# team-charls/charls

Hardware: AMD Instinct MI355X
Metric: MPixels/s encode+decode, 4096x4096 8-bit gray, bit-exact vs CharLS (higher is better)
Workload: dtype u8

## Files before the change

charls_amd/csrc/device/scan_group_decode.hip:

```cpp
#pragma once
#include <hip/hip_runtime.h>

#include "scan_model.h"
#include "scan_fast_decode.hip"
#ifndef JLS_EMULATED
#include "scan_group_step.inc"
#endif

namespace jls {
namespace grp {

constexpr uint32_t kRingWords = 256;
constexpr uint32_t kRingBits = kRingWords * 32;
constexpr int kStepsPerCheck = 64;
constexpr uint32_t kMarginBits = kStepsPerCheck * 32 + 320;
constexpr int kMaxTableT3 = 1023;
constexpr uint32_t kPrepRing = 128;
constexpr uint32_t kPrepSlots = kPrepRing + 64;
constexpr uint32_t kPrepChunk = 64;
constexpr int kStepsPerLoop = 63;

template <typename S>
struct Layout
{
    static constexpr uint32_t kLutBytes = sizeof(S) == 1 ? 512 : 2 * kMaxTableT3 + 2;
    static constexpr uint32_t kRecords = 0;
    static constexpr uint32_t kRun = 2928;
    static constexpr uint32_t kRing = kRun + 48;
    static constexpr uint32_t kPrep = kRing + kRingWords * 4 + 8;
    static constexpr uint32_t kLine = kPrep + kPrepSlots * 8 + 24 + 16 - sizeof(S);
    static_assert(kPrep % 8 == 0 && (kLine + sizeof(S)) % 16 == 0, "alignment of the prepared entries and of sample 1 of the line");
};

__host__ __device__ constexpr uint32_t bank_spread(uint32_t bytes)
{
    return ((bytes + 127u) & ~127u) + 16u;
}

template <typename S>
__host__ __device__ constexpr uint32_t line_stride_bytes(uint32_t width)
{
    return ((width + 6) * (uint32_t)sizeof(S) + 15u) & ~15u;
}

template <typename S>
__host__ __device__ constexpr uint32_t region_bytes(uint32_t width, uint32_t lines = 1)
{
    return bank_spread(Layout<S>::kLine + lines * line_stride_bytes<S>(width));
}

template <typename S>
__host__ __device__ constexpr uint32_t workgroup_lds_bytes(uint32_t width, uint32_t scans_per_wave, uint32_t lines = 1)
{
    return Layout<S>::kLutBytes + scans_per_wave * region_bytes<S>(width, lines);
}

struct Record
{
    uint32_t a;
    uint32_t ncb;
};

struct PrepEntry
{
    uint32_t x, y;
};
JLS_DEV PrepEntry load_pair(uint32_t address)
{
    const uint64_t w = lds_load<uint64_t>(address);
    return PrepEntry{(uint32_t)w, (uint32_t)(w >> 32)};
}
JLS_DEV void store_pair(uint32_t address, const PrepEntry& e)
{
    lds_store<uint64_t>(address, ((uint64_t)e.y << 32) | e.x);
}

#ifndef JLS_EMULATED
JLS_DEV uint32_t abs_difference_plus(uint32_t a, uint32_t b, uint32_t c)
{
    uint32_t r;
    asm("v_sad_u32 %0, %1, %2, %3" : "=v"(r) : "v"(a), "v"(b), "v"(c));
    return r;
}
#else
JLS_DEV uint32_t abs_difference_plus(uint32_t a, uint32_t b, uint32_t c)
{
    return (a > b ? a - b : b - a) + c;
}
#endif

JLS_DEV uint32_t peek32(const uint32_t* ring, uint32_t p)
{
    const uint32_t wi = (p >> 5) & (kRingWords - 1);
    const uint64_t both = ((uint64_t)ring[wi + 1] << 32) | ring[wi];
    return (uint32_t)(both >> (p & 31));
}

JLS_DEV uint64_t ring_words_at(uint32_t ring_address, uint32_t p)
{
    const uint32_t at = ring_address + (bit_field(p, 5, 8) << 2);
    return ((uint64_t)lds_load<uint32_t>(at + 4) << 32) | lds_load<uint32_t>(at);
}

JLS_DEV uint32_t field(uint32_t w, int n)
{
    return (uint32_t)(((uint64_t)bit_reverse(w) << n) >> 32);
}

JLS_DEV uint32_t take_bits(const uint32_t* ring, uint32_t& p, int n)
{
    const uint32_t w = peek32(ring, p);
    p += (uint32_t)n;
    return field(w, n);
}

struct Producer
{
    const uint8_t* gbase;
    uint64_t u_next;
    uint64_t u_end;
    uint64_t u_begin;
    uint64_t u_marker;
    uint32_t produced;
    uint32_t prev_byte;
    bool ended;
};

JLS_DEV void put_bits(uint32_t* ring, uint32_t p, uint32_t v, int n)
{
    const uint32_t q = (p >> 5) & (kRingWords - 1);
    const int off = (int)(p & 31);
    const uint32_t rv = bit_reverse(v) >> (32 - n);
    atomicOr(&ring[q], rv << off);
    if (q < 2)
        atomicOr(&ring[kRingWords + q], rv << off);
    if (off + n > 32)
    {
        const uint32_t q2 = (q + 1) & (kRingWords - 1);
        atomicOr(&ring[q2], rv >> (32 - off));
        if (q2 < 2)
            atomicOr(&ring[kRingWords + q2], rv >> (32 - off));
    }
}

template <int G>
JLS_DEV void refill_bytewise(Producer& s, uint32_t* ring, bool want, int lane, int sub, uint64_t u0, const uint4& raw,
                             uint32_t next_first, uint32_t before)
{
    constexpr uint32_t kChunk = G * 16;
    const uint32_t words[4] = {raw.x, raw.y, raw.z, raw.w};
    const uint32_t last = words[3] >> 24;
    int nbits[16];
    uint32_t bytes[16];
    int marker_at = 16;
    uint32_t prev = before;
    int total = 0;
#pragma unroll
    for (int j = 0; j < 16; ++j)
    {
        const uint32_t b = (words[j >> 2] >> ((j & 3) * 8)) & 0xFFu;
        const uint64_t u = u0 + (uint64_t)j;
        bytes[j] = b;
        int n = 0;
        if (u == s.u_begin)
            prev = 0;
        if (want && u >= s.u_begin && u < s.u_end && marker_at == 16)
        {
            const uint32_t nb = j < 15 ? ((words[(j + 1) >> 2] >> (((j + 1) & 3) * 8)) & 0xFFu) : next_first;
            const bool is_marker = b == 0xFFu && (u + 1 >= s.u_end || (nb & 0x80u) != 0);
            if (is_marker)
                marker_at = j;
            else
                n = prev == 0xFFu ? 7 : 8;
        }
        nbits[j] = n;
        total += n;
        prev = b;
    }
    const unsigned long long markers = __ballot(marker_at < 16);
    const int group_base = lane - sub;
    const uint32_t group_markers = (uint32_t)(markers >> group_base) & (G == 32 ? 0xFFFFFFFFu : ((1u << (G & 31)) - 1u));
    const unsigned long long group_markers64 = G == 64 ? markers : (unsigned long long)group_markers;
    const int first_marker = group_markers64 ? __ffsll(group_markers64) - 1 : 64;
    if (sub > first_marker)
        total = 0;
    int inc = total;
    for (int delta = 1; delta < G; delta <<= 1)
    {
        const int up = __shfl_up(inc, delta);
        if (sub >= delta)
            inc += up;
    }
    uint32_t p = s.produced + (uint32_t)(inc - total);
    if (want && sub <= first_marker)
    {
#pragma unroll
        for (int j = 0; j < 16; ++j)
            if (nbits[j] != 0)
            {
                put_bits(ring, p, nbits[j] == 7 ? (bytes[j] & 0x7Fu) : bytes[j], nbits[j]);
                p += (uint32_t)nbits[j];
            }
    }
    const int chunk_bits = __shfl(inc, group_base + G - 1);
    const uint32_t chunk_last = __shfl(last, group_base + G - 1);
    const int marker_j = __shfl(marker_at, group_base + (first_marker < G ? first_marker : 0));
    JLS_LOCKSTEP();
    if (want)
    {
        s.produced += (uint32_t)chunk_bits;
        s.prev_byte = chunk_last;
        if (first_marker < G)
        {
            s.u_marker = s.u_next + (uint64_t)first_marker * 16 + (uint64_t)marker_j;
            s.ended = true;
        }
        s.u_next += kChunk;
        if (s.u_next >= s.u_end)
            s.ended = true;
    }
}

JLS_DEV uint32_t ff_bytes(uint32_t w)
{
    const uint32_t v = ~w;
    return ~((((v & 0x7F7F7F7Fu) + 0x7F7F7F7Fu) | v) | 0x7F7F7F7Fu);
}

template <int G>
JLS_DEV void refill(Producer& s, uint32_t* ring, bool want, int lane, int sub)
{
    constexpr uint32_t kChunk = G * 16;
    if (want)
    {
        const uint32_t first = (s.produced + 31) >> 5;
        for (uint32_t j = sub; j < kChunk / 4 + 2; j += G)
        {
            const uint32_t q = (first + j) & (kRingWords - 1);
            ring[q] = 0;
            if (q < 2)
                ring[kRingWords + q] = 0;
        }
    }
    JLS_LOCKSTEP();
    const uint64_t u0 = s.u_next + (uint64_t)sub * 16;
    uint4 raw = make_uint4(0, 0, 0, 0);
    uint32_t next_first = 0;
    if (want && u0 < s.u_end)
    {
        raw = *reinterpret_cast<const uint4*>(s.gbase + u0);
        if (u0 + 16 < s.u_end)
            next_first = s.gbase[u0 + 16];
    }
    const uint32_t last = raw.w >> 24;
    uint32_t before = __shfl_up(last, 1);
    if (sub == 0)
        before = s.prev_byte;
    const uint32_t z0 = ff_bytes(raw.x), z1 = ff_bytes(raw.y), z2 = ff_bytes(raw.z), z3 = ff_bytes(raw.w);
    const uint32_t marker_like = (((z0 << 8) & raw.x) | (((z1 << 8) | (z0 >> 24)) & raw.y) | (((z2 << 8) | (z1 >> 24)) & raw.z) |
                                  (((z3 << 8) | (z2 >> 24)) & raw.w) | ((z3 >> 24) & next_first)) & 0x80808080u;
    const bool inside = u0 >= s.u_begin && u0 + 17 <= s.u_end;
    if (!__all(!want || (inside && marker_like == 0)))
    {
        JLS_PATH(11);
        refill_bytewise<G>(s, ring, want, lane, sub, u0, raw, next_first, before);
        return;
    }
    uint32_t d0 = __builtin_bswap32(bit_reverse(raw.x)), d1 = __builtin_bswap32(bit_reverse(raw.y));
    uint32_t d2 = __builtin_bswap32(bit_reverse(raw.z)), d3 = __builtin_bswap32(bit_reverse(raw.w));
    uint32_t f0 = (((z0 << 8) | (before == 0xFFu ? 0x80u : 0u))) >> 7, f1 = ((z1 << 8) | (z0 >> 24)) >> 7;
    uint32_t f2 = ((z2 << 8) | (z1 >> 24)) >> 7, f3 = ((z3 << 8) | (z2 >> 24)) >> 7;
    const int total = want ? 128 - (__popc(f0) + __popc(f1) + __popc(f2) + __popc(f3)) : 0;
    if (!want)
        f0 = f1 = f2 = f3 = 0;
    while (__any((f0 | f1 | f2 | f3) != 0))
    {
        JLS_PATH(12);
        if ((f0 | f1 | f2 | f3) != 0)
        {
            const int at = f3 ? 3 : (f2 ? 2 : (f1 ? 1 : 0));
            const uint32_t fw = f3 ? f3 : (f2 ? f2 : (f1 ? f1 : f0));
            const uint32_t bit = 31u - leading_zeros(fw);
            const uint32_t below = (1u << bit) - 1u;
            const uint32_t e0 = (d0 >> 1) | (d1 << 31), e1 = (d1 >> 1) | (d2 << 31), e2 = (d2 >> 1) | (d3 << 31), e3 = d3 >> 1;
            d0 = at == 0 ? (d0 & below) | (e0 & ~below) : d0;
            d1 = at == 1 ? (d1 & below) | (e1 & ~below) : (at < 1 ? e1 : d1);
            d2 = at == 2 ? (d2 & below) | (e2 & ~below) : (at < 2 ? e2 : d2);
            d3 = at == 3 ? (d3 & below) | (e3 & ~below) : e3;
            f0 = at == 0 ? f0 & below : f0;
            f1 = at == 1 ? f1 & below : f1;
            f2 = at == 2 ? f2 & below : f2;
            f3 = at == 3 ? f3 & below : f3;
        }
    }
    int inc = total;
    for (int delta = 1; delta < G; delta <<= 1)
    {
        const int up = __shfl_up(inc, delta);
        if (sub >= delta)
            inc += up;
    }
    const int group_base = lane - sub;
    if (want)
    {
        const uint32_t p = s.produced + (uint32_t)(inc - total);
        const uint32_t o = p & 31u;
        const uint32_t q = p >> 5;
        const uint32_t c[5] = {d0 << o, (uint32_t)((((uint64_t)d1 << 32) | d0) << o >> 32), (uint32_t)((((uint64_t)d2 << 32) | d1) << o >> 32),
                               (uint32_t)((((uint64_t)d3 << 32) | d2) << o >> 32), (uint32_t)(((uint64_t)d3 << o) >> 32)};
#pragma unroll
        for (int j = 0; j < 5; ++j)
        {
            const uint32_t qj = (q + (uint32_t)j) & (kRingWords - 1);
            atomicOr(&ring[qj], c[j]);
            if (qj < 2)
                atomicOr(&ring[kRingWords + qj], c[j]);
        }
    }
    const int chunk_bits = __shfl(inc, group_base + G - 1);
    const uint32_t chunk_last = __shfl(last, group_base + G - 1);
    JLS_LOCKSTEP();
    if (want)
    {
        s.produced += (uint32_t)chunk_bits;
        s.prev_byte = chunk_last;
        s.u_next += kChunk;
        if (s.u_next >= s.u_end)
            s.ended = true;
    }
}

JLS_DEV uint32_t run_prefix(uint32_t r)
{
    const uint32_t fours = ((4u + (r & 3u)) << (r >> 2)) - 4u;
    const uint32_t twos = 28u + ((2u + (r & 1u)) << (4u + (((r - 16u) >> 1) & 7u)));
    const uint32_t ones = 284u + (1u << ((r - 16u) & 31u));
    return r <= 16u ? fours : (r <= 24u ? twos : ones);
}

JLS_DEV int take_unary(const uint32_t* ring, uint32_t& p, int most)
{
    int total = 0;
    for (;;)
    {
        const uint32_t w = peek32(ring, p);
        const int u = w == 0 ? 32 : __ffs((int)w) - 1;
        if (u < 32)
        {
            p += (uint32_t)(u + 1);
            total += u;
            return total > most ? -1 : total;
        }
        p += 32;
        total += 32;
        if (total > most)
            return -1;
    }
}

}

template <typename S, int G, int NL = 1, int W = 1, bool kNear = false>
__global__ void __launch_bounds__(64 * W) decode_scans_group(const ScanDesc* __restrict__ descs, ScanResult* __restrict__ results,
                                                             uint32_t count)
{
    using namespace grp;
    using L = Layout<S>;
    static_assert(G == 4 || G == 8 || G == 16 || G == 32, "lanes per scan");
    static_assert(NL >= 1 && NL <= 4, "lines per pixel row");
    static_assert(W == 1 || W == 2 || W == 4 || W == 8, "wavefronts per workgroup");
    constexpr int kScansPerWave = 64 / G;
    constexpr bool kWide = sizeof(S) > 1;
    constexpr bool kChecked = kWide || kNear;
    JLS_DYNAMIC_LDS(smem);
    const int lane = W == 1 ? (int)threadIdx.x : (int)(threadIdx.x & 63u);
    const int wave = W == 1 ? 0 : (int)(threadIdx.x >> 6);
    const int sid = lane / G;
    const int sub = lane % G;
    const uint32_t scan = (blockIdx.x * (uint32_t)W + (uint32_t)wave) * kScansPerWave + (uint32_t)sid;
    const bool live = scan < count;
    const ScanDesc d = descs[live ? scan : count - 1];
    const Traits t = make_traits(d);
    const uint32_t width = d.width;

    unsigned char* region = smem + L::kLutBytes + (size_t)(wave * kScansPerWave + sid) * region_bytes<S>(width, NL);
    Record* records = reinterpret_cast<Record*>(region + L::kRecords);
    RunCtx* run_ctx = reinterpret_cast<RunCtx*>(region + L::kRun);
    uint32_t* ring = reinterpret_cast<uint32_t*>(region + L::kRing);
    const uint32_t ring_address = opaque(lds_address(ring));
    unsigned char* lut = smem;
    const ScanDesc& d_first = descs[blockIdx.x * (uint32_t)(W * kScansPerWave)];
    const Traits t_first = make_traits(d_first);
    S* const line0 = reinterpret_cast<S*>(region + L::kLine);
    const uint32_t line_stride = line_stride_bytes<S>(width) / (uint32_t)sizeof(S);
    S* line = line0;
    const int cap = kWide ? t_first.t3 : 255;
    const bool own_table = t.t1 == t_first.t1 && t.t2 == t_first.t2 && t.t3 == t_first.t3 && t.bpp == t_first.bpp && t.near == t_first.near &&
                           (t.near != 0) == kNear;

    {
        const Record fresh{(uint32_t)initial_a(t), 1u};
        for (int q = sub; q < 366; q += G)
            records[q] = q == 0 ? Record{fresh.a, (uint32_t)t.reset} : fresh;
        if (sub < 2)
            run_ctx[sub] = RunCtx{sub, initial_a(t), 1, 0};
        for (int q = (int)threadIdx.x; q <= 2 * cap && q < (int)L::kLutBytes; q += 64 * W)
            lut[q] = (unsigned char)((quantize(t_first, q - cap) + 4) * 8);
        for (uint32_t q = sub; q < (NL == 1 ? width + 6 : NL * line_stride); q += G)
            line0[q] = 0;
        for (uint32_t q = sub; q <= kRingWords + 1; q += G)
            ring[q] = 0;
    }
    Producer src;
    {
        const uint64_t mis = (uint64_t)(reinterpret_cast<uintptr_t>(d.stream) & 15u);
        src.gbase = d.stream - mis;
        src.u_begin = mis;
        src.u_next = 0;
        src.u_end = mis + d.stream_capacity;
        src.u_marker = ~0ull;
        src.produced = 0;
        src.prev_byte = 0;
        src.ended = d.stream_capacity == 0;
    }
    if (W > 1)
        __syncthreads();
    JLS_LOCKSTEP();

    enum : int { kLineStart = 0, kInLine, kDrain, kDone };
    const bool usable = own_table && (!kWide || t_first.t3 <= kMaxTableT3) && lds_address(smem) == 0;
    int phase = !live || !usable ? kDone : (d.height == 0 ? kDrain : kLineStart);
    bool retry = live && !usable;
    uint32_t p = 0;
    uint32_t y = 0, i = 1;
    int corner = 0, first = 0, run_index = 0;
    int comp = 0;
    int corner_of[NL], run_index_of[NL];
#pragma unroll
    for (int c = 0; c < NL; ++c)
        corner_of[c] = run_index_of[c] = 0;
    int a = 0;
    uint32_t a_seen = 0;
    const int maxval = t.maxval, reset = t.reset;
    const uint32_t limit_m = (uint32_t)(t.limit - t.qbpp - 1);
    constexpr int kLongestPrefix = kNear ? 62 : 47;
    const int near = kNear ? t.near : 0, near_step = 2 * near + 1, range_step = t.range * near_step;
    auto same_level = [&](int ra, int rb) -> bool { return kNear ? abs_difference((uint32_t)ra, (uint32_t)rb) <= (uint32_t)near : ra == rb; };
    auto reconstructed = [&](int predicted, int e) -> int {
        if (!kNear)
            return (predicted + e) & maxval;
        int v = mad24(e, near_step, predicted);
        v += v < -near ? range_step : (v > maxval + near ? -range_step : 0);
        return med3(v, 0, maxval);
    };
    auto interruption_sample = [&](bool which, int ra, int rb, int e) -> int {
        return which ? reconstructed(ra, e) : reconstructed(rb, (rb - ra) < 0 ? -e : e);
    };
    const uint32_t records_address = lds_address(records);
    const uint32_t prep_address = lds_address(region + L::kPrep);
    uint32_t prepped_end = 0;
    int rc_over = 0;

    auto quantised = [&](int diff) -> int {
        if (kWide)
            diff = med3(diff, -cap, cap);
        return (int)lds_load<unsigned char>((uint32_t)(diff + cap));
    };
    auto prepare = [&](bool want, uint32_t from, bool first_is_over) {
        constexpr uint32_t kPer = kPrepChunk / G;
        const uint32_t j0 = from + (uint32_t)sub * kPer;
        const uint32_t last = width + 1;
        int v[kPer + 2];
#pragma unroll
        for (uint32_t c = 0; c < kPer + 2; ++c)
        {
            const uint32_t at = j0 - 1 + c;
            v[c] = (int)line[at < last ? at : last];
        }
        if (first_is_over && sub == 0)
            v[0] = rc_over;
        int g[kPer + 1];
#pragma unroll
        for (uint32_t c = 0; c < kPer + 1; ++c)
            g[c] = quantised(v[c + 1] - v[c]);
        JLS_LOCKSTEP();
#pragma unroll
        for (uint32_t c = 0; c < kPer; ++c)
        {
            const uint32_t j = j0 + c;
            const uint32_t tt = (uint32_t)mad24(g[c + 1], 81, 9 * g[c]);
            const uint32_t slot = j & (kPrepRing - 1);
            const PrepEntry entry{(uint32_t)v[c] | (tt << 16), (uint32_t)v[c + 1]};
            if (want && j <= width)
            {
                store_pair(prep_address + slot * 8u, entry);
                if (slot < kPrepSlots - kPrepRing)
                    store_pair(prep_address + (slot + kPrepRing) * 8u, entry);
            }
        }
        JLS_LOCKSTEP();
    };

    for (;;)
    {
        JLS_PATH(0);
        const bool look = !__all(phase == kDone || (phase == kInLine && (src.ended || src.produced - p >= kMarginBits)));
        {
            const uint32_t ahead = src.produced - p;
            const bool busy = phase != kDone && !src.ended;
            const bool need = busy && (phase == kDrain ? ahead < 64u : ahead < kMarginBits);
            if (look && __any(need))
            {
                const bool want = busy && ahead <= kRingBits - G * 128u - 128u;
                JLS_PATH(1);
                refill<G>(src, ring, want, lane, sub);
                continue;
            }
        }
        {
            const bool starting = phase == kLineStart;
            if (look && __any(starting))
            {
                JLS_PATH(2);
                if (NL > 1 && starting)
                {
                    line = line0 + (uint32_t)comp * line_stride;
#pragma unroll
                    for (int c = 0; c < NL; ++c)
                    {
                        corner = comp == c ? corner_of[c] : corner;
                        run_index = comp == c ? run_index_of[c] : run_index;
                    }
                }
                if (starting && sub == 0)
                    line[width + 1] = line[width];
                JLS_LOCKSTEP();
                if (starting)
                {
                    i = 1;
                    prepped_end = 0;
                    rc_over = corner;
                    a = (int)line[1];
                    first = a;
                    phase = kInLine;
                }
            }
        }
        {
            const uint32_t reach = i + (uint32_t)kStepsPerLoop < width ? i + (uint32_t)kStepsPerLoop : width;
            const bool need = phase == kInLine && prepped_end < reach;
            if (__any(need))
            {
                JLS_PATH(14);
                const uint32_t from = prepped_end + 1 > i ? prepped_end + 1 : i;
                prepare(need, from, from == i);
                if (need)
                    prepped_end = from + kPrepChunk - 1;
            }
        }
        const bool in_line = phase == kInLine;
        const LaneMask in_line_m = lanes_where(in_line);
        LaneMask ok_m = ~0ull;
        uint32_t qsu8 = 2912;
        uint32_t win_stopped = 0;
        PrepEntry entry_stopped{0, 0};
        if (in_line_m != 0)
        {
            const uint32_t rest_of_line = width + 1 - i;
            uint32_t steps = kStepsPerLoop;
            for (;;)
            {
                const LaneMask closer = lanes_where(in_line && rest_of_line < steps);
                if (closer == 0)
                    break;
                JLS_PATH(4);
                steps = value_of_lowest_lane(closer, rest_of_line);
            }
            JLS_PATH(3);
            const uint32_t limit_v = opaque(in_line ? limit_m : 0u);
            const uint32_t p_kept = p;
            constexpr uint32_t kSz = (uint32_t)sizeof(S);
            const uint32_t line_address = lds_address(line);
            uint32_t lm = in_line ? line_address + (i - 2) * kSz : line_address + (width + 1) * kSz;
            uint32_t pp = prep_address + ((i & (kPrepRing - 1)) << 3) - (in_line ? 8u : 0u);
            uint32_t where = records_address + 365u * 8u;
            int u_a = 0, u_n1 = 2, u_tb = 0, u_cc = 0;
            uint32_t u1 = 0, k_last = 0, t_mm = 0;
            uint32_t k_seen = 0, mm_seen = 0, a_seen_now = 0;
            uint32_t win_now = 0;
#if defined(JLS_EMULATED) || defined(JLS_CXX_STEP_LOOP)
            const uint32_t lm_step = in_line ? kSz : 0u;
            const uint32_t pp_step = in_line ? 8u : 0u;
            uint64_t ticker = 1ull << (steps - 1);
            const uint32_t pp_first = pp + 8u;
            do
            {
                JLS_PATH(5);
                p += u1 + k_last;
                if (kChecked)
                    mm_seen |= t_mm;
                lm += lm_step;
                pp += pp_step;
                const PrepEntry entry = load_pair(pp);
                const uint64_t ring_words = ring_words_at(ring_address, p);
                const int rc = kWide ? (int)(entry.x & 0xFFFFu) : (int)(entry.x & 0xFFu);
                const int rb = (int)entry.y;
                const int q3 = quantised(rc - a);
                Record updated;
                {
                    const int n_new = u_n1;
                    const int minus_delta = 1 - med3(u_tb, 0, 1) - med3(u_tb + n_new, 0, 1);
                    const int b_new = med3(mad24(minus_delta, n_new, u_tb), 1 - n_new, 0);
                    const int c_new = med3(u_cc - minus_delta, -128, 127);
                    updated = Record{(uint32_t)u_a, ((uint32_t)b_new << 16) | pack_bytes((uint32_t)c_new, (uint32_t)n_new)};
                }
                const uint32_t win = (uint32_t)(ring_words >> (p & 31));
                win_now = win;
                qsu8 = (entry.x >> 16) + (uint32_t)q3;
                const uint32_t here = abs_difference_plus(qsu8, 2912u, records_address);
                const int sgn = qsu8 < 2912u ? -1 : 1;
                JLS_LOCKSTEP();
                store_pair(where, PrepEntry{updated.a, updated.ncb});
                lds_store<S>(lm, (S)a);
                JLS_LOCKSTEP();
                where = here;
                const PrepEntry rec = load_pair(here);
                const uint32_t u = lowest_one(win);
                u1 = u + 1u;
                const uint32_t beyond = bit_reverse(win >> (u1 & 31u));
                const int px0 = med3(a + (rb - rc), a, rb);
                ok_m = lanes_where(qsu8 != 2912u) & lanes_where(u < limit_v);
                const int n = (int)(rec.y & 0xFFu);
                const int cc = (int)(signed char)(rec.y >> 8);
                const int bb = (int)rec.y >> 16;
                const int k_raw = ((int)(float_bits(rec.x) - float_bits((uint32_t)n)) + 0x7FFFFF) >> 23;
                const int k = k_raw < 0 ? 0 : k_raw;
                if (kChecked)
                    ok_m &= lanes_where(u + (uint32_t)k < 32u);
                const int mm = (int)(uint32_t)(((((uint64_t)u << 32) | beyond) << (k & 63)) >> 32);
                const int half = (int)(((uint32_t)mm >> 1) & 0x1FFFFu);
                const int odd = kNear ? (mm & 1) : ((mm ^ (int)((uint32_t)((k - 1) & (2 * bb + n - 1)) >> 31)) & 1);
                const int e = half ^ -odd;
                const int px = med3(mad24(cc, sgn, px0), 0, maxval);
                int e_scaled = e;
                if (kNear)
                {
                    e_scaled = mad24(e, near_step, 0);
                    int v = mad24(e, sgn < 0 ? -near_step : near_step, px);
                    v += v < -near ? range_step : (v > maxval + near ? -range_step : 0);
                    a = med3(v, 0, maxval);
                }
                else
                    a = mad24(e, sgn, px) & maxval;
                k_last = (uint32_t)k;
                t_mm = (uint32_t)mm;
                u_a = (int)rec.x + half + odd;
                if (kChecked)
                    a_seen_now |= (uint32_t)u_a;
                u_n1 = n + 1;
                u_tb = bb + e_scaled;
                u_cc = cc;
                if (n == reset)
                {
                    u_a >>= 1;
                    u_n1 = (n >> 1) + 1;
                    u_tb >>= 1;
                }
                k_seen |= (uint32_t)k;
                {
                    const LaneMask run_m = in_line_m & lanes_where(qsu8 == 2912u);
                    const LaneMask unusual_m = in_line_m & ~(lanes_where(u < limit_v) & (kChecked ? lanes_where(u + (uint32_t)k < 32u) : ~0ull));
                    if (run_m != 0 && unusual_m == 0)
                    {
                        const bool mine = lane_of(run_m);
                        const RunCtx ctx0 = run_ctx[0], ctx1 = run_ctx[1];
                        const int ra = (int)lds_load<S>(lm);
                        const uint32_t ones = lowest_one(~win);
                        const uint32_t ri2 = (uint32_t)run_index + ones;
                        bool fits = mine && ones <= 16u && ri2 <= 16u;
                        const uint32_t j = fits ? ri2 >> 2 : 0u;
                        const uint32_t blocks = fits ? ((4u + (ri2 & 3u)) << j) - ((4u + ((uint32_t)run_index & 3u)) << ((uint32_t)run_index >> 2)) : 0u;
                        const uint32_t run = blocks + field(fits ? win >> (ones + 1u) : 0u, (int)j);
                        const uint32_t used = fits ? ones + 1u + j : 0u;
                        const uint32_t taken = ((pp - pp_first) >> 3) + run + 1u;
                        const uint32_t budget = rest_of_line < (uint32_t)kStepsPerLoop ? rest_of_line : (uint32_t)kStepsPerLoop;
                        fits = fits && run <= (uint32_t)G && taken <= budget;
                        const int rb = (int)lds_load<S>(lm + ((fits ? run : 0u) + 1u) * kSz);
                        const int which = same_level(ra, rb) ? 1 : 0;
                        RunCtx ctx = which ? ctx1 : ctx0;
                        const uint32_t goal = (uint32_t)ctx.a + (uint32_t)(ctx.n >> 1) * (uint32_t)ctx.ritype;
                        int kr = 0;
                        if (goal > (uint32_t)ctx.n)
                        {
                            kr = (int)leading_zeros((uint32_t)ctx.n) - (int)leading_zeros(goal);
                            kr += (((uint64_t)(uint32_t)ctx.n << kr) < goal) ? 1 : 0;
                        }
                        const uint32_t w3 = win >> used;
                        const uint32_t zeros = lowest_one(w3);
                        const int escape_from = t.limit - (int)j - 1 - t.qbpp - 1;
                        const int tail_bits = (int)zeros < escape_from ? kr : t.qbpp;
                        const uint32_t event_bits = used + zeros + 1u + (uint32_t)tail_bits;
                        fits = fits && kr <= 24 && zeros < 32u && event_bits <= 32u;
                        const LaneMask served_m = lanes_where(fits);
                        if (served_m != 0)
                        {
                            JLS_PATH(16);
                            const uint32_t tail = field(fits ? w3 >> ((zeros + 1u) & 31u) : 0u, fits ? tail_bits : 0);
                            const int em = (int)zeros < escape_from ? ((int)zeros << kr) + (int)tail : (int)tail + 1;
                            const int er = run_error_value(ctx, em + ctx.ritype, kr);
                            run_update(ctx, er, em, t.reset);
                            const int x = interruption_sample(which != 0, ra, rb, er);
                            JLS_LOCKSTEP();
                            if (fits)
                            {
                                if ((uint32_t)sub < run)
                                    lds_store<S>(lm + ((uint32_t)sub + 1u) * kSz, (S)ra);
                                run_ctx[which] = ctx;
                                a = x;
                                u1 = event_bits;
                                k_last = 0;
                                t_mm = 0;
                                where = records_address + 365u * 8u;
                                run_index = ri2 > 0 ? (int)ri2 - 1 : 0;
                                lm += run * kSz;
                                pp += run * 8u;
                            }
                            JLS_LOCKSTEP();
                            ok_m |= served_m;
                            const uint32_t may_take = fits ? budget - taken : ~0u;
                            uint32_t left = 63u - (uint32_t)__builtin_clzll(ticker);
                            for (LaneMask m = served_m; m != 0;)
                            {
                                const uint32_t v = value_of_lowest_lane(m, may_take);
                                left = v < left ? v : left;
                                m &= ~lanes_where(may_take == v);
                            }
                            ticker = 1ull << left;
                        }
                    }
                }
                ticker = tick(ticker, in_line_m, ok_m);
            } while (ticker != 0);
#else
            {
                LaneMask fail_m;
                uint32_t count = steps - 1;
                const int cap_v = cap;
                const uint32_t run_ctx_address = lds_address(run_ctx);
                const uint32_t cfg_v = (uint32_t)(t.limit - t.qbpp - 2) | ((uint32_t)t.qbpp << 8) | ((uint32_t)reset << 16);
                const int maxval_s = (int)uniform((uint32_t)maxval);
                lds_store<uint64_t>(run_ctx_address + 32u, ((uint64_t)rest_of_line << 32) | (uint64_t)(pp + 8u));
                [[maybe_unused]] const int near_range_s = (int)uniform((uint32_t)near | ((uint32_t)range_step << 8));
                if constexpr (kNear && kWide)
                    JLS_STEP_LOOP_ASM_WIDE_NEAR();
                else if constexpr (kNear)
                    JLS_STEP_LOOP_ASM_NARROW_NEAR();
                else if constexpr (kWide)
                    JLS_STEP_LOOP_ASM_WIDE();
                else
                    JLS_STEP_LOOP_ASM_NARROW();
                (void)cap_v;
                ok_m = in_line_m & ~fail_m;
            }
#endif
            win_stopped = win_now;
            bool owed_last;
            int ra_stopped;
            {
                RegCtx ctx{u_a, u_tb, u_cc, u_n1};
                const int minus_delta = 1 - med3(ctx.b, 0, 1) - med3(ctx.b + ctx.n, 0, 1);
                ctx.b = med3(ctx.b + minus_delta * ctx.n, 1 - ctx.n, 0);
                ctx.c = med3(ctx.c - minus_delta, -128, 127);
                const bool owed = in_line && lane_of(ok_m);
                owed_last = owed;
                JLS_LOCKSTEP();
                ra_stopped = (int)lds_load<S>(lm);
                if (owed)
                {
                    store_pair(where, PrepEntry{(uint32_t)ctx.a, ((uint32_t)ctx.b << 16) | pack_bytes((uint32_t)ctx.c, (uint32_t)ctx.n)});
                    lm += kSz;
                    lds_store<S>(lm, (S)a);
                    p += u1 + k_last;
                    if (kChecked)
                        mm_seen |= t_mm;
                }
                JLS_LOCKSTEP();
            }
            if (in_line)
            {
                if (!owed_last)
                    a = ra_stopped;
                i = (lm - line_address) / kSz + 1;
                a_seen |= a_seen_now;
                if (k_seen >= (kChecked ? 16u : 10u) || (kChecked && mm_seen > 131071u))
                    retry = true;
            }
            else
                p = p_kept;
            if (in_line && !owed_last)
                entry_stopped = load_pair(pp);
        }
        const int qs8 = (int)qsu8 - 2912;
        const bool stopped = in_line && !lane_of(ok_m);
        const bool in_run = stopped && qs8 == 0 && !retry;
        const bool slow = stopped && qs8 != 0 && !retry;
        if (in_line_m != 0 && __all(phase == kDone || (in_line && !stopped && !retry && i <= width && !(kChecked && a_seen >= (1u << 24)))))
            continue;

        bool windowed_runs = false;
        if (__any(in_run))
        {
            const uint32_t remaining = width - (i - 1);
            const uint32_t wi = (p >> 5) & (kRingWords - 1);
            const uint32_t r0 = ring[wi], r1 = ring[wi + 1], r2 = ring[wi + 2];
            const RunCtx ctx0 = run_ctx[0], ctx1 = run_ctx[1];
            const uint32_t lo = funnel_shift(r1, r0, p), hi = funnel_shift(r2, r1, p);
            const uint64_t w = ((uint64_t)hi << 32) | lo;
            const uint32_t ones = lowest_one(~lo);
            const uint32_t ri_after = (uint32_t)run_index + ones;
            const bool counted = ones < 32u && ri_after <= 31u;
            const uint32_t ri2 = counted ? ri_after : 0u;
            const uint32_t blocks = run_prefix(ri2) - run_prefix((uint32_t)run_index);
            const int j = run_j((int)ri2);
            const uint32_t after_zero = (uint32_t)(w >> ((ones + 1u) & 63u));
            const uint32_t run = blocks + field(after_zero, j);
            const uint32_t used = ones + 1u + (uint32_t)j;
            const bool inside = counted && blocks < remaining && run < remaining;
            const uint32_t at = inside ? i + run : i;
            JLS_LOCKSTEP();
            const int b_at = (int)line[at];
            const int which = same_level(a, b_at) ? 1 : 0;
            RunCtx ctx = which ? ctx1 : ctx0;
            const uint32_t goal = (uint32_t)ctx.a + (uint32_t)(ctx.n >> 1) * (uint32_t)ctx.ritype;
            int k = 0;
            if (goal > (uint32_t)ctx.n)
            {
                k = (int)leading_zeros((uint32_t)ctx.n) - (int)leading_zeros(goal);
                k += (((uint64_t)(uint32_t)ctx.n << k) < goal) ? 1 : 0;
            }
            const uint32_t w3 = (uint32_t)(w >> (used & 63u));
            const uint32_t zeros = lowest_one(w3);
            const int escape_from = t.limit - j - 1 - t.qbpp - 1;
            const int tail_bits = (int)zeros < escape_from ? k : t.qbpp;
            const uint32_t code_bits = zeros + 1u + (uint32_t)tail_bits;
            const bool fits = inside && k <= 24 && zeros < 32u && used + code_bits <= 64u;
            windowed_runs = __all(!in_run || fits);
            if (windowed_runs)
            {
                JLS_PATH(15);
                const uint32_t tail = field((uint32_t)(w >> ((used + zeros + 1u) & 63u)), tail_bits);
                const int em = (int)zeros < escape_from ? ((int)zeros << k) + (int)tail : (int)tail + 1;
                const int e = run_error_value(ctx, em + ctx.ritype, k);
                run_update(ctx, e, em, t.reset);
                const int x = interruption_sample(which != 0, a, b_at, e);
                JLS_LOCKSTEP();
                {
                    uint32_t r = (uint32_t)sub;
                    while (__any(in_run && r < run))
                    {
                        JLS_PATH(8);
                        if (in_run && r < run)
                            line[i + r] = (S)a;
                        r += G;
                    }
                }
                JLS_LOCKSTEP();
                if (in_run)
                {
                    run_ctx[which] = ctx;
                    line[at] = (S)x;
                    a = x;
                    run_index = ri2 > 0 ? (int)ri2 - 1 : 0;
                    i = at + 1;
                    p += used + code_bits;
                    rc_over = b_at;
                }
                JLS_LOCKSTEP();
            }
        }
        if (!windowed_runs && __any(in_run))
        {
            JLS_PATH(6);
            const uint32_t remaining = width - (i - 1);
            uint32_t run = 0;
            uint32_t window = peek32(ring, p);
            uint32_t used = 0;
            bool counting = in_run && (window & 1u) != 0;
            if (in_run && !counting)
            {
                window >>= 1;
                used = 1;
            }
            while (__any(counting))
            {
                JLS_PATH(7);
                if (counting)
                {
                    if (used == 32)
                    {
                        p += 32;
                        used = 0;
                        window = peek32(ring, p);
                    }
                    const uint32_t bit = window & 1u;
                    window >>= 1;
                    ++used;
                    if (bit)
                    {
                        const uint32_t block = 1u << run_j(run_index);
                        const uint32_t count_now = block < remaining - run ? block : remaining - run;
                        run += count_now;
                        if (count_now == block && run_index < 31)
                            ++run_index;
                        if (run == remaining)
                            counting = false;
                    }
                    else
                        counting = false;
                }
            }
            bool interrupted = in_run && run != remaining;
            if (interrupted)
            {
                const int j = run_j(run_index);
                if (used + (uint32_t)j <= 32)
                {
                    run += field(window, j);
                    used += (uint32_t)j;
                }
                else
                {
                    p += used;
                    used = 0;
                    run += take_bits(ring, p, j);
                }
                if (run > remaining)
                {
                    retry = true;
                    interrupted = false;
                    run = 0;
                }
            }
            if (in_run)
                p += used;
            JLS_LOCKSTEP();
            {
                uint32_t r = (uint32_t)sub;
                while (__any(in_run && r < run))
                {
                    JLS_PATH(8);
                    if (in_run && r < run)
                        line[i + r] = (S)a;
                    r += G;
                }
            }
            const uint32_t at = i + run;
            JLS_LOCKSTEP();
            const int b_at = (int)line[interrupted ? at : 0];
            const int which = same_level(a, b_at) ? 1 : 0;
            RunCtx ctx = run_ctx[which];
            int x = 0;
            if (interrupted)
            {
                const uint32_t goal = (uint32_t)ctx.a + (uint32_t)(ctx.n >> 1) * (uint32_t)ctx.ritype;
                int k = 0;
                if (goal > (uint32_t)ctx.n)
                {
                    k = (int)leading_zeros((uint32_t)ctx.n) - (int)leading_zeros(goal);
                    k += (((uint64_t)(uint32_t)ctx.n << k) < goal) ? 1 : 0;
                }
                const int limit = t.limit - run_j(run_index) - 1;
                const uint32_t w2 = peek32(ring, p);
                const uint32_t zeros = lowest_one(w2);
                int u = -1;
                int em = 0;
                if (k <= 24 && zeros < 32u)
                {
                    u = (int)zeros;
                    const int tail_bits = u < limit - t.qbpp - 1 ? k : t.qbpp;
                    uint32_t tail;
                    if (zeros + 1u + (uint32_t)tail_bits <= 32u)
                    {
                        tail = field(zeros == 31u ? 0u : w2 >> (zeros + 1u), tail_bits);
                        p += zeros + 1u + (uint32_t)tail_bits;
                    }
                    else
                    {
                        p += zeros + 1u;
                        tail = take_bits(ring, p, tail_bits);
                    }
                    em = u < limit - t.qbpp - 1 ? (u << k) + (int)tail : (int)tail + 1;
                }
                else if (k <= 24)
                {
                    u = take_unary(ring, p, kLongestPrefix);
                    if (u >= 0)
                    {
                        if (u < limit - t.qbpp - 1)
                            em = (u << k) + (int)take_bits(ring, p, k);
                        else
                            em = (int)take_bits(ring, p, t.qbpp) + 1;
                    }
                }
                if (u < 0)
                {
                    retry = true;
                    interrupted = false;
                }
                else
                {
                    const int e = run_error_value(ctx, em + ctx.ritype, k);
                    run_update(ctx, e, em, t.reset);
                    x = interruption_sample(which != 0, a, b_at, e);
                }
            }
            JLS_LOCKSTEP();
            if (interrupted)
            {
                run_ctx[which] = ctx;
                line[at] = (S)x;
                a = x;
                if (run_index > 0)
                    --run_index;
                i = at + 1;
                rc_over = b_at;
            }
            else if (in_run && !retry)
                i = width + 1;
            JLS_LOCKSTEP();
        }

        if (__any(slow))
        {
            JLS_PATH(9);
            const int rc = kWide ? (int)(entry_stopped.x & 0xFFFFu) : (int)(entry_stopped.x & 0xFFu), rb = (int)entry_stopped.y;
            const int s = qs8 >> 31;
            const int idx = ((qs8 ^ s) - s) >> 3;
            const Record rec = records[idx];
            RegCtx ctx{(int)rec.a, (int)rec.ncb >> 16, (int)(signed char)(rec.ncb >> 8), (int)(rec.ncb & 0xFFu)};
            const int k = regular_k(ctx);
            const int px = clamp_sample(t, med_predict(a, rb, rc) + ((ctx.c ^ s) - s));
            int x = 0;
            bool good = slow && k < 16;
            if (good)
            {
                const int u = take_unary(ring, p, kLongestPrefix);
                if (u < 0)
                    good = false;
                else
                {
                    int mm;
                    if ((uint32_t)u < limit_m)
                        mm = (u << k) | (int)take_bits(ring, p, k);
                    else
                        mm = (int)take_bits(ring, p, t.qbpp) + 1;
                    int e = unmap_error(mm);
                    if (k == 0)
                        e ^= error_correction(ctx, near);
                    if (!regular_update(ctx, e, near, t.reset))
                        good = false;
                    x = reconstructed(px, (e ^ s) - s);
                }
            }
            JLS_LOCKSTEP();
            if (good)
            {
                records[idx] = Record{(uint32_t)ctx.a,
                                      (uint32_t)ctx.n | (((uint32_t)ctx.c & 0xFFu) << 8) | ((uint32_t)ctx.b << 16)};
                line[i] = (S)x;
                a = x;
                ++i;
                rc_over = rb;
            }
            else if (slow)
                retry = true;
            JLS_LOCKSTEP();
        }

        if (kChecked && a_seen >= (1u << 24))
            retry = true;
        if (retry)
            phase = kDone;

        if (NL == 1)
        {
            const bool ending = phase == kInLine && i > width;
            if (__any(ending))
            {
                JLS_PATH(10);
                uint8_t* row = d.pixels + (size_t)y * d.pixel_stride;
                const S* samples = line + 1;
                const uint32_t row_bytes = width * (uint32_t)sizeof(S);
                const bool aligned = ((reinterpret_cast<uintptr_t>(d.pixels) | d.pixel_stride) & 15u) == 0;
                const uint32_t wide_bytes = aligned ? row_bytes & ~15u : 0u;
                uint32_t off = (uint32_t)sub * 16u;
                while (__any(ending && off < wide_bytes))
                {
                    if (ending && off < wide_bytes)
                        *reinterpret_cast<uint4*>(row + off) =
                            *reinterpret_cast<const uint4*>(reinterpret_cast<const uint8_t*>(samples) + off);
                    off += G * 16u;
                }
                uint32_t xx = wide_bytes / (uint32_t)sizeof(S) + (uint32_t)sub;
                while (__any(ending && xx < width))
                {
                    if (ending && xx < width)
                        reinterpret_cast<S*>(row)[xx] = samples[xx];
                    xx += G;
                }
                JLS_LOCKSTEP();
                if (ending)
                {
                    corner = first;
                    ++y;
                    phase = y == d.height ? kDrain : kLineStart;
                }
            }
        }
        else
        {
            const bool ending = phase == kInLine && i > width;
            if (__any(ending))
            {
                const bool row_done = ending && comp == NL - 1;
                if (__any(row_done))
                {
                    uint8_t* row = d.pixels + (size_t)y * d.pixel_stride;
                    const bool transformed = NL == 3 && d.color_transformation != 0;
                    uint32_t xx = (uint32_t)sub;
                    while (__any(row_done && xx < width))
                    {
                        if (row_done && xx < width)
                        {
                            unsigned v[4];
#pragma unroll
                            for (int c = 0; c < NL; ++c)
                                v[c] = line0[(uint32_t)c * line_stride + 1 + xx];
                            if (transformed)
                                hp_inverse(d.color_transformation, kWide, (int)v[0], (int)v[1], (int)v[NL > 2 ? 2 : 0], v);
#pragma unroll
                            for (int c = 0; c < NL; ++c)
                            {
                                uint8_t* q = row + ((size_t)xx * NL + c) * sizeof(S);
                                q[0] = (uint8_t)v[c];
                                if (kWide)
                                    q[1] = (uint8_t)(v[c] >> 8);
                            }
                        }
                        xx += G;
                    }
                }
                JLS_LOCKSTEP();
                if (ending)
                {
#pragma unroll
                    for (int c = 0; c < NL; ++c)
                    {
                        corner_of[c] = comp == c ? first : corner_of[c];
                        run_index_of[c] = comp == c ? run_index : run_index_of[c];
                    }
                    if (comp == NL - 1)
                    {
                        comp = 0;
                        ++y;
                    }
                    else
                        ++comp;
                    phase = y == d.height ? kDrain : kLineStart;
                }
            }
        }
        {
            const bool draining = phase == kDrain;
            const uint32_t ahead = src.produced - p;
            if (draining && (src.ended || ahead >= 64u))
                phase = kDone;
        }
        if (__all(phase == kDone))
            break;
    }

    ScanResult r{kOk, 0, 0};
    if (!retry)
    {
        const uint32_t left = src.produced - p;
        const bool clean = src.u_marker != ~0ull && left < 15u && (left == 0 || field(peek32(ring, p), (int)left) == 0);
        if (clean)
            r.bytes = src.u_marker - src.u_begin;
        else
            retry = true;
    }
    if (retry)
        r.flags = fast::kFastRetry;
    if (live && sub == 0)
        results[scan] = r;
}

}
```

charls_amd/csrc/device/scan_group_step.inc:

```

#define JLS_SDWA(s0, s1) " dst_sel:DWORD dst_unused:UNUSED_PAD src0_sel:" s0 " src1_sel:" s1 "\n"

#define JLS_STEP_PROLOGUE                                                                                                          \
    "s_mov_b64 s[98:99], exec\n"                                                                                                  \
    "s_mov_b64 exec, %[inl]\n"                                                                                                    \
    "ds_read_b64 v[118:119], %[pp] offset:8\n"                                                                                    \
    "v_mov_b32 v100, 0xb60\n"                                                                                                     \
    "v_mov_b32 v101, 0x0c0c0400\n"                                                                                                \
    "v_mov_b32 v103, 0x7f\n"                                                                                                      \
    "v_mov_b32 v104, 0xffffff80\n"                                                                                                \
    "v_mov_b32 v105, 1\n"                                                                                                         \
    "v_mov_b32 v127, 0\n"                                                                                                         \
    "v_lshrrev_b32 v93, 16, %[cfg]\n"                                                                                 \
    "s_waitcnt lgkmcnt(0)\n"

#define JLS_STEP_STORES_LATE(ST) "ds_write2_b32 %[where], %[ua], v111 offset1:1\n", "2", ST " %[lm], %[a]\n", "1"
#define JLS_STEP_STORES_EARLY(ST) "ds_write2_b32 %[where], %[ua], v111 offset1:1\n" ST " %[lm], %[a]\n", "3", "", "0"

#define JLS_STEP_COMMIT_AND_WINDOW(SZ, TOP_EXTRA) \
     \
    "v_add3_u32 %[p], %[p], %[u1], %[k]\n" \
    "v_add_u32 %[lm], " SZ ", %[lm]\n" \
    "v_add_u32 %[pp], 8, %[pp]\n" \
    TOP_EXTRA \
    "v_bfe_u32 v109, %[p], 5, 8\n" \
    "v_lshl_add_u32 v109, v109, 2, %[ring]\n" \
    "ds_read2_b32 v[120:121], v109 offset1:1\n"
#define JLS_STEP_PREDICTOR(RC, E0, E1) \
     \
    "v_add_u32 v115, %[a], " E1 "\n" \
    "v_sub_u32_sdwa v115, v115, " E0 JLS_SDWA("DWORD", RC) \
    "v_med3_i32 v115, v115, %[a], " E1 "\n"
#define JLS_STEP_A13 \
     \
    "v_med3_i32 v110, %[utb], 0, 1\n" \
    "v_add_u32 v111, %[utb], %[un1]\n" \
    "v_med3_i32 v111, v111, 0, 1\n" \
    "v_add_u32 v110, v110, v111\n" \
    "v_sub_u32 v110, 1, v110\n" \
    "v_sub_u32 v111, %[cc], v110\n" \
    "v_mad_i32_i24 v112, v110, %[un1], %[utb]\n" \
    "v_med3_i32 v111, v111, v104, v103\n" \
    "v_sub_u32 v113, 1, %[un1]\n" \
    "v_med3_i32 v112, v112, v113, 0\n" \
    "v_perm_b32 v111, v111, %[un1], v101\n" \
    "v_lshl_or_b32 v111, v112, 16, v111\n"

#define JLS_STEP_ODD_LOSSLESS                                                                                                      \
    "v_add_u32_sdwa v109, v123, sext(v123)" JLS_SDWA("BYTE_0", "WORD_1")                                                          \
    "v_add_u32_sdwa v109, v109, sext(v123)" JLS_SDWA("DWORD", "WORD_1")                                                           \
    "v_add_u32 v109, -1, v109\n"                                                                                                  \
    "v_add_u32 v110, -1, %[k]\n"                                                                                                  \
    "v_and_b32 v109, v109, v110\n"                                                                                                \
    "v_lshrrev_b32 v109, 31, v109\n"                                                                                              \
    "v_bitop3_b32 v109, v127, 1, v109 bitop3:0x48\n"
#define JLS_STEP_RECON_LOSSLESS                                                                                                    \
    "v_mad_i32_i24 v115, v111, v116, v115\n"                                                                                      \
    "v_and_b32 %[a], %[smax], v115\n"
#define JLS_STEP_LOSSLESS "", JLS_STEP_ODD_LOSSLESS, JLS_STEP_RECON_LOSSLESS, "v111"
#define JLS_STEP_RECON_NEAR                                                                                                        \
    "v_mad_i32_i24 v115, v111, v117, v115\n"                                                                                      \
    "v_cmp_lt_i32 vcc, v115, v96\n"                                                                                               \
    "v_cmp_gt_i32 s[88:89], v115, v97\n"                                                                                          \
    "v_mul_i32_i24 v112, v111, v94\n"                                                                                             \
    "v_cndmask_b32 v113, 0, v98, vcc\n"                                                                                           \
    "v_cndmask_b32_e64 v113, v113, v99, s[88:89]\n"                                                                               \
    "v_add_u32 v115, v115, v113\n"                                                                                                \
    "v_med3_i32 %[a], v115, 0, %[smax]\n"
#define JLS_STEP_NEAR "v_cndmask_b32 v117, v94, v95, vcc\n", "v_and_b32 v109, 1, v127\n", JLS_STEP_RECON_NEAR, "v112"
#define JLS_STEP_NEAR_CONSTANTS                                                                                                    \
    "s_and_b32 s80, %[nr], 0xff\n"                                                                                     \
    "s_lshr_b32 s81, %[nr], 8\n"                                                                         \
    "v_lshl_add_u32 v94, s80, 1, 1\n"                                                                                             \
    "v_sub_u32 v96, 0, s80\n"                                                                                                     \
    "v_mov_b32 v98, s81\n"                                                                                                        \
    "v_sub_u32 v95, 0, v94\n"                                                                                                     \
    "v_sub_u32 v97, %[smax], v96\n"                                                                                               \
    "v_sub_u32 v99, 0, v98\n"

#define JLS_STEP_BODY(SFX, NEXT, E0, E1, ENEXT, RC, SZ, BETWEEN, RING_WAIT, AFTER_REQUEST, EARLY_STORES, Q3_WAIT, LATE_STORE, RECORD_WAIT, Q3_ADDR, Q3_OFFSET, TOP_EXTRA, K_EXTRA, A_EXTRA, KSEEN, SIGN_EXTRA, ODD, RECON, UTB_SRC) \
    "L_step" SFX "%=:\n"                                                                                                          \
                                                                \
    "v_sub_u32_sdwa v108, " E0 ", %[a]" JLS_SDWA(RC, "DWORD")                                                                    \
    Q3_ADDR                                                                                                                       \
    "ds_read_u8 v114, v108" Q3_OFFSET "\n"                                                                            \
    BETWEEN                                                                                                                       \
    EARLY_STORES                                                                                                \
    "s_waitcnt lgkmcnt(" Q3_WAIT ")\n"                                                                           \
    "v_add_u32_sdwa %[qsu], v114, " E0 JLS_SDWA("DWORD", "WORD_1")                                                                \
    "ds_read_b64 " ENEXT ", %[pp] offset:8\n"                                \
    "v_sad_u32 %[where], %[qsu], v100, %[recbase]\n"                                                                              \
    "ds_read_b64 v[122:123], %[where]\n"                                                                 \
    LATE_STORE                                                                                                                    \
    AFTER_REQUEST                                                                                                                 \
    "v_cmp_gt_u32 vcc, v100, %[qsu]\n"                                                                                            \
    "s_waitcnt lgkmcnt(" RING_WAIT ")\n"                                                            \
    "v_alignbit_b32 %[win], v121, v120, %[p]\n"                                                                                   \
    "v_ffbl_b32 v125, %[win]\n"                                                                                                   \
    "v_cndmask_b32_e64 v116, 1, -1, vcc\n"                                                              \
    SIGN_EXTRA                                                                                                                    \
    "v_add_u32 %[u1], 1, v125\n"                                                                                                  \
    "v_lshrrev_b32 v124, %[u1], %[win]\n"                                                                                         \
    "v_bfrev_b32 v124, v124\n"                                                                                                    \
    "v_cmp_ge_u32 s[96:97], v125, %[limitv]\n"                                       \
    "s_waitcnt lgkmcnt(" RECORD_WAIT ")\n"                                                               \
    "v_cmp_eq_u32_sdwa s[92:93], v123, v93 src0_sel:BYTE_0 src1_sel:DWORD\n"           \
                            \
    "v_cvt_f32_u32 v108, v122\n"                                                                                                  \
    "v_cvt_f32_ubyte0 v109, v123\n"                                                                                               \
    "v_add_u32 v108, 0x7fffff, v108\n"                                                                                            \
    "v_sub_u32_e64 v108, v108, v109 clamp\n"                                                                                      \
    "v_lshrrev_b32 %[k], 23, v108\n"                                                                                              \
    "v_lshlrev_b64 v[126:127], %[k], v[124:125]\n"                                                      \
    K_EXTRA                                                                                                                       \
    ODD                                                                         \
    "v_bfe_u32 v110, v127, 1, 17\n"                                          \
    "v_sub_u32 v111, 0, v109\n"                                                                                                   \
    "v_xor_b32 v111, v110, v111\n"                                                                                   \
    "v_bfe_i32 %[cc], v123, 8, 8\n"                                                                                               \
    "v_mad_i32_i24 v115, %[cc], v116, v115\n"                                                                                     \
    "v_med3_i32 v115, v115, 0, %[smax]\n"                                                                                         \
    RECON                                                                                                        \
                                                                          \
    "v_add3_u32 %[ua], v122, v110, v109\n"                                                                                        \
    A_EXTRA                                                                                                                       \
    "v_add_u32_sdwa %[un1], v123, v105" JLS_SDWA("BYTE_0", "DWORD")                                                               \
    "v_add_u32_sdwa %[utb], " UTB_SRC ", sext(v123)" JLS_SDWA("DWORD", "WORD_1")                                                  \
    KSEEN                                                                                                                         \
    "s_or_b64 s[94:95], s[92:93], s[96:97]\n"                                                    \
    "s_cbranch_scc1 L_rare" SFX "%=\n"                                                                                            \
    "L_back" SFX "%=:\n"                                                                                                          \
    "s_sub_u32 %[cnt], %[cnt], 1\n"                                                                                               \
    "s_cbranch_scc1 L_done%=\n"                                                             \
    NEXT

#define JLS_RUN_WHICH_LOSSLESS "v_cmp_eq_u32 s[88:89], v108, v109\n"
#define JLS_RUN_WHICH_NEAR                                                                                                         \
    "v_sad_u32 v91, v108, v109, v96\n"                                                                     \
    "v_cmp_ge_i32 s[88:89], 0, v91\n"
#define JLS_RUN_RECON_LOSSLESS                                                                                                     \
    "v_add_u32 v112, v112, v114\n"                                                                                                \
    "v_and_b32 v112, %[smax], v112\n"
#define JLS_RUN_RECON_NEAR                                                                                                         \
    "v_mad_i32_i24 v112, v114, v94, v112\n"                                                                                       \
    "v_cmp_lt_i32 vcc, v112, v96\n"                                                                                               \
    "v_cmp_gt_i32 s[86:87], v112, v97\n"                                                                                          \
    "s_nop 1\n"                                                                                                                   \
    "v_cndmask_b32 v91, 0, v98, vcc\n"                                                                                            \
    "v_cndmask_b32_e64 v91, v91, v99, s[86:87]\n"                                                                                 \
    "v_add_u32 v112, v112, v91\n"                                                                                                 \
    "v_med3_i32 v112, v112, 0, %[smax]\n"
#define JLS_STEP_RARE(SFX, LD, ST, SZ, ENEXT, WHICH, RECON)                                                                        \
    "L_rare" SFX "%=:\n"                                                                                                          \
    "v_cndmask_b32_e64 v108, 0, 1, s[92:93]\n"                                                                                    \
    "v_and_b32 v109, 0xff, v123\n"                                                                                                \
    "v_cmp_eq_u32 s[94:95], %[where], %[recbase]\n"                                                       \
    "v_ashrrev_i32 %[ua], v108, %[ua]\n"                                                                                          \
    "v_ashrrev_i32 %[utb], v108, %[utb]\n"                                                                                        \
    "v_lshrrev_b32 v109, v108, v109\n"                                                                                            \
    "v_add_u32 %[un1], 1, v109\n"                                                                                                 \
    "s_or_b64 %[fail], s[96:97], s[94:95]\n"                                                                                      \
    "s_cbranch_scc0 L_back" SFX "%=\n"                                                              \
    "s_cmp_lg_u64 s[96:97], 0\n"                                                                                                  \
    "s_cbranch_scc1 L_exit%=\n"                                              \
                                                                                   \
    "s_mov_b64 s[90:91], exec\n"                                                                                                  \
    "s_mov_b64 exec, s[94:95]\n"                                                                                                  \
    "ds_read_b128 v[120:123], %[rctx]\n"                                           \
    "ds_read_b128 v[124:127], %[rctx] offset:16\n"                                                                                \
    "ds_read_b64 v[116:117], %[rctx] offset:32\n"                            \
    LD " v108, %[lm]\n"                                                                                                  \
                            \
    "v_not_b32 v80, %[win]\n"                                                                                                     \
    "v_ffbl_b32 v80, v80\n"                                                        \
    "v_add_u32 v81, %[ri], v80\n"                                                                \
    "v_lshrrev_b32 v110, 2, v81\n"                                                                       \
    "v_and_b32 v82, 3, v81\n"                                                                                                     \
    "v_add_u32 v82, 4, v82\n"                                                                                                     \
    "v_lshlrev_b32 v82, v110, v82\n"                                                                                              \
    "v_and_b32 v83, 3, %[ri]\n"                                                                                                   \
    "v_lshrrev_b32 v84, 2, %[ri]\n"                                                                                               \
    "v_add_u32 v83, 4, v83\n"                                                                                                     \
    "v_lshlrev_b32 v83, v84, v83\n"                                                                                               \
    "v_sub_u32 v82, v82, v83\n"                                                              \
    "v_add_u32 v83, 1, v80\n"                                                                                                     \
    "v_lshrrev_b32 v84, v83, %[win]\n"                                                             \
    "v_bfrev_b32 v84, v84\n"                                                                                                      \
    "v_mov_b32 v85, 0\n"                                                                                                          \
    "v_cmp_ge_u32 s[82:83], 16, v80\n"                                                                \
    "v_cmp_ge_u32 s[84:85], 16, v81\n"                                                   \
    "v_lshlrev_b64 v[84:85], v110, v[84:85]\n"                                                             \
    "v_add_u32 v82, v82, v85\n"                                                                                         \
    "v_add_u32 v111, v83, v110\n"                                                               \
    "s_and_b64 s[84:85], s[84:85], s[82:83]\n"                                                                                    \
    "v_mad_u32_u24 v86, v82, " SZ ", %[lm]\n"                                            \
    LD " v109, v86 offset:" SZ "\n"                                           \
                     \
    "v_mbcnt_lo_u32_b32 v87, -1, 0\n"                                                                                             \
    "v_mbcnt_hi_u32_b32 v87, -1, v87\n"                                                                                           \
    "v_and_b32 v87, %[gl] - 1, v87\n"                                                 \
    "v_cmp_ge_u32 s[82:83], %[gl], v82\n"                                                                                         \
    "s_and_b64 s[84:85], s[84:85], s[82:83]\n"                                                                                    \
    "s_waitcnt lgkmcnt(2)\n"                                                           \
    "v_sub_u32 v88, %[pp], v116\n"                                                                                                \
    "v_lshrrev_b32 v88, 3, v88\n"                                                     \
    "v_add_u32 v88, v88, v82\n"                                                                                                   \
    "v_add_u32 v88, 1, v88\n"                                                                               \
    "v_min_u32 v89, 63, v117\n"                                                                                                   \
    "v_cmp_le_u32 s[82:83], v88, v89\n"                                      \
    "v_sub_u32 v89, v89, v88\n"                                                \
    "s_and_b64 s[84:85], s[84:85], s[82:83]\n"                                                                                    \
                                                                               \
    "v_lshrrev_b32 v113, v111, %[win]\n"                                                                                          \
    "v_ffbl_b32 v114, v113\n"                                                                           \
    "v_add_u32 v115, 1, v114\n"                                                                                                   \
    "v_lshrrev_b32 v116, v115, v113\n"                                                                                            \
    "v_bfrev_b32 v116, v116\n"                                                 \
    "v_and_b32 v117, 0xff, %[cfg]\n"                                                                                              \
    "v_sub_u32 v117, v117, v110\n"                                                     \
    "v_bfe_u32 v90, %[cfg], 8, 8\n"                                                                                    \
    "s_waitcnt lgkmcnt(0)\n"                                                                                                      \
    WHICH                                                                                 \
    "v_cmp_lt_u32 s[86:87], v114, v117\n"                                                    \
    "v_cmp_gt_u32 s[82:83], 32, v114\n"                                                                                           \
    "v_cndmask_b32_e64 v120, v120, v124, s[88:89]\n"                                                                              \
    "v_cndmask_b32_e64 v121, v121, v125, s[88:89]\n"                                                                              \
    "v_cndmask_b32_e64 v122, v122, v126, s[88:89]\n"                                                                              \
    "v_cndmask_b32_e64 v123, v123, v127, s[88:89]\n"                                                                              \
    "s_and_b64 s[84:85], s[84:85], s[82:83]\n"                                                                                    \
                                                 \
    "v_lshrrev_b32 v124, 1, v122\n"                                                                                               \
    "v_mul_u32_u24 v124, v124, v120\n"                                                                                            \
    "v_add_u32 v124, v121, v124\n"                                                                                                \
    "v_max_u32 v125, 1, v124\n"                                                                                                   \
    "v_ffbh_u32 v125, v125\n"                                                                                                     \
    "v_ffbh_u32 v126, v122\n"                                                                                                     \
    "v_sub_u32 v125, v126, v125\n"                                                                                                \
    "v_max_i32 v125, 0, v125\n"                                                                                                   \
    "v_lshlrev_b32 v126, v125, v122\n"                                                                                            \
    "v_cmp_lt_u32 vcc, v126, v124\n"                                                                                              \
    "v_mov_b32 v112, v116\n"                                                                                                      \
    "v_mov_b32 v113, 0\n"                                                                                                         \
    "v_addc_co_u32 v125, vcc, 0, v125, vcc\n"                                                                             \
    "v_cndmask_b32_e64 v126, v90, v125, s[86:87]\n"                             \
    "v_add_u32 v127, v115, v126\n"                                                                                                \
    "v_add_u32 v111, v111, v127\n"                                                                  \
    "v_cmp_ge_u32 vcc, 24, v125\n"                                                                                                \
    "v_cmp_ge_u32 s[80:81], 32, v111\n"                                                         \
    "v_lshlrev_b64 v[112:113], v126, v[112:113]\n"                                                        \
    "s_and_b64 s[84:85], s[84:85], vcc\n"                                                                                         \
    "s_and_b64 s[84:85], s[84:85], s[80:81]\n"                                                        \
    "v_lshlrev_b32 v116, v125, v114\n"                                                                                            \
    "v_add_u32 v116, v116, v113\n"                                                                                                \
    "v_add_u32 v112, 1, v113\n"                                                                                                   \
    "v_cndmask_b32_e64 v116, v112, v116, s[86:87]\n"                                                               \
             \
                                                                                   \
    "v_add_u32 v112, v116, v120\n"                                                                                                \
    "v_and_b32 v113, 1, v112\n"                                                                                                   \
    "v_add_u32 v112, v112, v113\n"                                                                                                \
    "v_lshrrev_b32 v112, 1, v112\n"                                                                                               \
    "v_lshlrev_b32 v114, 1, v123\n"                                                                                               \
    "v_cmp_ge_u32 vcc, v114, v122\n"                                                                                              \
    "v_min_u32 v114, 1, v125\n"                                                                                                   \
    "s_nop 0\n"                                                                                                                   \
    "v_cndmask_b32_e64 v114, v114, 1, vcc\n"                                                                                      \
    "v_xor_b32 v114, v114, v113\n"                                                                                                \
    "v_add_u32 v114, -1, v114\n"                                                                \
    "v_xor_b32 v112, v112, v114\n"                                                                                                \
    "v_sub_u32 v112, v112, v114\n"                                                                                   \
                                                                                \
    "v_lshrrev_b32 v113, 31, v112\n"                                                                                              \
    "v_add_u32 v123, v123, v113\n"                                                                                                \
    "v_sub_u32 v113, v116, v120\n"                                                                                                \
    "v_add_u32 v113, 1, v113\n"                                                                                                   \
    "v_lshrrev_b32 v113, 1, v113\n"                                                                                               \
    "v_add_u32 v121, v121, v113\n"                                                                                                \
    "v_xor_b32 v113, v122, v93\n"                                                                                                 \
    "v_sub_u32_e64 v113, 1, v113 clamp\n"                                                                 \
    "v_lshrrev_b32 v121, v113, v121\n"                                                                                            \
    "v_lshrrev_b32 v123, v113, v123\n"                                                                                            \
    "v_lshrrev_b32 v122, v113, v122\n"                                                                                            \
    "v_add_u32 v122, 1, v122\n"                                                                                                   \
     \
    "v_sub_u32 v113, v109, v108\n"                                                                                                \
    "v_ashrrev_i32 v113, 31, v113\n"                                                                                              \
    "v_xor_b32 v114, v112, v113\n"                                                                                                \
    "v_sub_u32 v114, v114, v113\n"                                                                     \
    "v_cndmask_b32_e64 v114, v114, v112, s[88:89]\n"                                                                              \
    "v_cndmask_b32_e64 v112, v109, v108, s[88:89]\n"                                              \
    RECON                                                                                                                         \
                                                                                                  \
    "s_andn2_b64 s[94:95], s[94:95], s[84:85]\n"                                                  \
    "s_mov_b64 exec, s[84:85]\n"                                                                                                  \
    "s_cbranch_execz L_unserved" SFX "%=\n"                                                                                       \
    "v_cmp_lt_u32 vcc, v87, v82\n"                                               \
    "v_mad_u32_u24 v87, v87, " SZ ", %[lm]\n"                                                                                     \
    "v_cndmask_b32_e64 v113, 0, 16, s[88:89]\n"                                                                                   \
    "v_add_u32 v113, %[rctx], v113\n"                                                                                             \
    "ds_write_b128 v113, v[120:123]\n"                                                                                            \
    "s_and_b64 exec, exec, vcc\n"                                                                                                 \
    ST " v87, v108 offset:" SZ "\n"                                                                                               \
    "s_mov_b64 exec, s[84:85]\n"                                                                                                  \
    "v_mov_b32 %[lm], v86\n"                                                      \
    "v_lshl_add_u32 %[pp], v82, 3, %[pp]\n"                                                                                       \
    "ds_read_b64 " ENEXT ", %[pp] offset:8\n"                                      \
    "v_mov_b32 %[a], v112\n"                                                                                                      \
    "v_mov_b32 %[u1], v111\n"                                                                                                     \
    "v_mov_b32 %[k], 0\n"                                                                                                         \
    "v_mov_b32 v127, 0\n"                                                                                                         \
    "v_add_u32 %[where], 0xb68, %[recbase]\n"                                                                    \
    "v_sub_u32_e64 %[ri], v81, 1 clamp\n"                                                         \
                                                        \
    "s_mov_b64 s[82:83], exec\n"                                                                                                  \
    "L_budget" SFX "%=:\n"                                                                                                        \
    "s_ff1_i32_b64 s80, s[82:83]\n"                                                                                               \
    "s_nop 3\n"                                                                 \
    "v_readlane_b32 s81, v89, s80\n"                                                                                              \
    "s_min_u32 %[cnt], %[cnt], s81\n"                                                                                             \
    "s_nop 0\n"                                                             \
    "v_cmp_ne_u32 vcc, s81, v89\n"                                                                                                \
    "s_and_b64 s[82:83], s[82:83], vcc\n"                                                                                         \
    "s_cbranch_scc1 L_budget" SFX "%=\n"                                                                                          \
    "L_unserved" SFX "%=:\n"                                                                                                      \
    "s_waitcnt lgkmcnt(0)\n"                                                                                                      \
    "s_mov_b64 exec, s[90:91]\n"                                                                                                  \
    "s_mov_b64 %[fail], s[94:95]\n"                                                                                               \
    "s_cmp_lg_u64 s[94:95], 0\n"                                                                                                  \
    "s_cbranch_scc0 L_back" SFX "%=\n"                                                                                            \
    "s_branch L_exit%=\n"

#define JLS_STEP_EPILOGUE(EXIT_EXTRA)                                                                                              \
    "L_done%=:\n"                                                                                                                 \
    "s_mov_b64 %[fail], 0\n"                                                                                                      \
    "L_exit%=:\n"                                                                                                                 \
    EXIT_EXTRA                                                                                                                    \
    "s_waitcnt lgkmcnt(0)\n"                                                 \
    "s_mov_b64 exec, s[98:99]\n"

#define JLS_STEP_ORDER_WINDOW_FIRST(RC, SZ, TOP_EXTRA, E0, E1) JLS_STEP_COMMIT_AND_WINDOW(SZ, TOP_EXTRA) JLS_STEP_PREDICTOR(RC, E0, E1) JLS_STEP_A13, "4", ""
#define JLS_STEP_ORDER_PREDICTOR_LATE(RC, SZ, TOP_EXTRA, E0, E1) JLS_STEP_COMMIT_AND_WINDOW(SZ, TOP_EXTRA) JLS_STEP_A13, "4", JLS_STEP_PREDICTOR(RC, E0, E1)
#define JLS_STEP_ORDER_UPDATE_FIRST(RC, SZ, TOP_EXTRA, E0, E1)                                                                     \
    JLS_STEP_A13 "ds_write2_b32 %[where], %[ua], v111 offset1:1\n" JLS_STEP_COMMIT_AND_WINDOW(SZ, TOP_EXTRA) JLS_STEP_PREDICTOR(RC, E0, E1), "3", ""
#define JLS_STEP_STORES_SAMPLE_LATE(ST) "", "2", ST " %[lm], %[a]\n", "1"
#define JLS_STEP_KSEEN "v_or_b32 %[kseen], %[kseen], %[k]\n"

#define JLS_STEP_BODY_X(...) JLS_STEP_BODY(__VA_ARGS__)
#define JLS_STEP_LOOP_TEXT(RC, SZ, LD, ORDER, STORES, Q3_ADDR, Q3_OFFSET, TOP_EXTRA, K_EXTRA, A_EXTRA, EXIT_EXTRA, MODE, RARE_A, RARE_B)     \
    JLS_STEP_PROLOGUE                                                                                                              \
    JLS_STEP_BODY_X("a", "", "v118", "v119", "v[106:107]", RC, SZ, ORDER(RC, SZ, TOP_EXTRA, "v118", "v119"), STORES, Q3_ADDR, Q3_OFFSET, TOP_EXTRA, \
                  K_EXTRA, A_EXTRA, JLS_STEP_KSEEN, MODE)                                                                          \
    JLS_STEP_BODY_X("b", "s_branch L_stepa%=\n", "v106", "v107", "v[118:119]", RC, SZ, ORDER(RC, SZ, TOP_EXTRA, "v106", "v107"), STORES, Q3_ADDR, \
                  Q3_OFFSET, TOP_EXTRA, K_EXTRA, A_EXTRA, JLS_STEP_KSEEN, MODE)                                                    \
    RARE_A                                                                                                                         \
    RARE_B                                                                                                                         \
    JLS_STEP_EPILOGUE(EXIT_EXTRA)

#define JLS_STEP_LOOP_CLOBBERS                                                                                                     \
    "memory", "vcc", "scc", "s80", "s81", "s82", "s83", "s84", "s85", "s86", "s87", "s88", "s89", "s90", "s91", "s92", "s93", "s94", "s95", "s96",   \
        "s97", "s98", "s99", "v80", "v81", "v82", "v83", "v84", "v85", "v86", "v87", "v88", "v89", "v90", "v91", "v92", "v93", "v94", "v95", "v96", "v97", "v98", "v99", "v100", "v101", "v102", "v103", "v104", "v105", "v106", "v107",      \
        "v108", "v109", "v110", "v111", "v112", "v113", "v114", "v115", "v116", "v117", "v118", "v119", "v120", "v121", "v122", "v123", "v124",  \
        "v125", "v126", "v127"

#define JLS_STEP_RARE_NARROW(SFX, ENEXT, WHICH, RECON) JLS_STEP_RARE(SFX, "ds_read_u8", "ds_write_b8", "1", ENEXT, WHICH, RECON)
#define JLS_STEP_RARE_WIDE(SFX, ENEXT, WHICH, RECON) JLS_STEP_RARE(SFX, "ds_read_u16", "ds_write_b16", "2", ENEXT, WHICH, RECON)
#define JLS_STEP_OPERANDS_OUT                                                                                                      \
    [a] "+v"(a), [p] "+v"(p), [lm] "+v"(lm), [pp] "+v"(pp), [where] "+v"(where), [ua] "+v"(u_a), [un1] "+v"(u_n1), [utb] "+v"(u_tb), \
        [cc] "+v"(u_cc), [u1] "+v"(u1), [k] "+v"(k_last), [kseen] "+v"(k_seen), [qsu] "+v"(qsu8), [win] "+v"(win_now),             \
        [cnt] "+s"(count), [fail] "=&s"(fail_m), [ri] "+v"(run_index)
#define JLS_STEP_OPERANDS_CHECKED , [mmseen] "+v"(mm_seen), [aseen] "+v"(a_seen_now), [tmm] "+v"(t_mm)
#define JLS_STEP_OPERANDS_IN                                                                                                       \
    [ring] "v"(ring_address), [recbase] "v"(records_address), [limitv] "v"(limit_v), [cfg] "v"(cfg_v), [inl] "s"(in_line_m),       \
        [smax] "s"(maxval_s), [rctx] "v"(run_ctx_address), [gl] "n"(G)

#define JLS_STEP_LOOP_ASM_NARROW()                                                                                                 \
    asm volatile(JLS_STEP_LOOP_TEXT("BYTE_0", "1", "ds_read_u8", JLS_STEP_ORDER_WINDOW_FIRST,                                      \
                                    JLS_STEP_STORES_LATE("ds_write_b8"), "", " offset:255", "", "", "", "", JLS_STEP_LOSSLESS,      \
                                    JLS_STEP_RARE_NARROW("a", "v[106:107]", JLS_RUN_WHICH_LOSSLESS, JLS_RUN_RECON_LOSSLESS), JLS_STEP_RARE_NARROW("b", "v[118:119]", JLS_RUN_WHICH_LOSSLESS, JLS_RUN_RECON_LOSSLESS))                          \
                 : JLS_STEP_OPERANDS_OUT                                                                                           \
                 : JLS_STEP_OPERANDS_IN                                                                                            \
                 : JLS_STEP_LOOP_CLOBBERS)

#define JLS_STEP_CHECKED_TOP "v_or_b32 %[mmseen], %[mmseen], v127\n"
#define JLS_STEP_CHECKED_K "v_add_u32 v112, v125, %[k]\n v_cmp_le_u32 vcc, 32, v112\n s_or_b64 s[96:97], s[96:97], vcc\n"
#define JLS_STEP_CHECKED_A "v_or_b32 %[aseen], %[aseen], %[ua]\n"
#define JLS_STEP_CHECKED_EXIT "v_mov_b32 %[tmm], v127\n"
#define JLS_STEP_WIDE_Q3 "v_med3_i32 v108, v108, v102, %[vcap]\n v_add_u32 v108, %[vcap], v108\n"
#define JLS_STEP_LOOP_ASM_WIDE()                                                                                                   \
    asm volatile("v_sub_u32 v102, 0, %[vcap]\n"                                                                                   \
                 JLS_STEP_LOOP_TEXT("WORD_0", "2", "ds_read_u16", JLS_STEP_ORDER_WINDOW_FIRST, JLS_STEP_STORES_LATE("ds_write_b16"), \
                                    JLS_STEP_WIDE_Q3, "", JLS_STEP_CHECKED_TOP, JLS_STEP_CHECKED_K, JLS_STEP_CHECKED_A,             \
                                    JLS_STEP_CHECKED_EXIT, JLS_STEP_LOSSLESS,                                                      \
                                    JLS_STEP_RARE_WIDE("a", "v[106:107]", JLS_RUN_WHICH_LOSSLESS, JLS_RUN_RECON_LOSSLESS), JLS_STEP_RARE_WIDE("b", "v[118:119]", JLS_RUN_WHICH_LOSSLESS, JLS_RUN_RECON_LOSSLESS))                            \
                 : JLS_STEP_OPERANDS_OUT JLS_STEP_OPERANDS_CHECKED                                                                 \
                 : JLS_STEP_OPERANDS_IN, [vcap] "v"(cap_v)                                                                         \
                 : JLS_STEP_LOOP_CLOBBERS)

#define JLS_STEP_LOOP_ASM_NARROW_NEAR()                                                                                            \
    asm volatile(JLS_STEP_NEAR_CONSTANTS                                                                                           \
                 JLS_STEP_LOOP_TEXT("BYTE_0", "1", "ds_read_u8", JLS_STEP_ORDER_WINDOW_FIRST, JLS_STEP_STORES_LATE("ds_write_b8"), \
                                    "", " offset:255", JLS_STEP_CHECKED_TOP, JLS_STEP_CHECKED_K, JLS_STEP_CHECKED_A,                \
                                    JLS_STEP_CHECKED_EXIT, JLS_STEP_NEAR, JLS_STEP_RARE_NARROW("a", "v[106:107]", JLS_RUN_WHICH_NEAR, JLS_RUN_RECON_NEAR), JLS_STEP_RARE_NARROW("b", "v[118:119]", JLS_RUN_WHICH_NEAR, JLS_RUN_RECON_NEAR)) \
                 : JLS_STEP_OPERANDS_OUT JLS_STEP_OPERANDS_CHECKED                                                                 \
                 : JLS_STEP_OPERANDS_IN, [nr] "s"(near_range_s)                                                                    \
                 : JLS_STEP_LOOP_CLOBBERS)
#define JLS_STEP_LOOP_ASM_WIDE_NEAR()                                                                                              \
    asm volatile("v_sub_u32 v102, 0, %[vcap]\n" JLS_STEP_NEAR_CONSTANTS                                                           \
                 JLS_STEP_LOOP_TEXT("WORD_0", "2", "ds_read_u16", JLS_STEP_ORDER_WINDOW_FIRST, JLS_STEP_STORES_LATE("ds_write_b16"), \
                                    JLS_STEP_WIDE_Q3, "", JLS_STEP_CHECKED_TOP, JLS_STEP_CHECKED_K, JLS_STEP_CHECKED_A,             \
                                    JLS_STEP_CHECKED_EXIT, JLS_STEP_NEAR, JLS_STEP_RARE_WIDE("a", "v[106:107]", JLS_RUN_WHICH_NEAR, JLS_RUN_RECON_NEAR), JLS_STEP_RARE_WIDE("b", "v[118:119]", JLS_RUN_WHICH_NEAR, JLS_RUN_RECON_NEAR)) \
                 : JLS_STEP_OPERANDS_OUT JLS_STEP_OPERANDS_CHECKED                                                                 \
                 : JLS_STEP_OPERANDS_IN, [vcap] "v"(cap_v), [nr] "s"(near_range_s)                                                 \
                 : JLS_STEP_LOOP_CLOBBERS)
```

Baseline: 17570.

## Compute median predictor relative to Ra and pair-unroll decode step loop

For 8-bit lossless scans, the prepared entries now pack Rc and Rb as bytes plus the difference Rb-Rc. The median predictor is then computed as Ra plus a clamped offset, using SDWA byte selects, so the per-step mask of the reconstructed value can be dropped when maxval is 255. The step loop is also unrolled in pairs with a halved trip counter and pointer advances folded into store offsets. This cuts scalar loop overhead and pointer arithmetic. It adds odd/even entry paths, budget rounding to whole pairs and extra code size in the hand-written asm.

```diff
diff --git a/charls_amd/csrc/device/scan_group_decode.hip b/charls_amd/csrc/device/scan_group_decode.hip
--- a/charls_amd/csrc/device/scan_group_decode.hip
+++ b/charls_amd/csrc/device/scan_group_decode.hip
@@ -19,6 +19,12 @@
 constexpr uint32_t kPrepSlots = kPrepRing + 64;
 constexpr uint32_t kPrepChunk = 64;
 constexpr int kStepsPerLoop = 63;
+#ifndef JLS_STEP_MED_FROM_RA
+#define JLS_STEP_MED_FROM_RA 1
+#endif
+#ifndef JLS_STEP_TRIP_COUNT
+#define JLS_STEP_TRIP_COUNT 1
+#endif
 
 template <typename S>
 struct Layout
@@ -372,6 +378,7 @@
     constexpr int kScansPerWave = 64 / G;
     constexpr bool kWide = sizeof(S) > 1;
     constexpr bool kChecked = kWide || kNear;
+    constexpr bool kRelative = JLS_STEP_MED_FROM_RA != 0 && !kWide;
     JLS_DYNAMIC_LDS(smem);
     const int lane = W == 1 ? (int)threadIdx.x : (int)(threadIdx.x & 63u);
     const int wave = W == 1 ? 0 : (int)(threadIdx.x >> 6);
@@ -490,7 +497,8 @@
             const uint32_t j = j0 + c;
             const uint32_t tt = (uint32_t)mad24(g[c + 1], 81, 9 * g[c]);
             const uint32_t slot = j & (kPrepRing - 1);
-            const PrepEntry entry{(uint32_t)v[c] | (tt << 16), (uint32_t)v[c + 1]};
+            const PrepEntry entry = kRelative ? PrepEntry{(uint32_t)v[c] | ((uint32_t)v[c + 1] << 8) | (tt << 16), (uint32_t)(v[c + 1] - v[c])}
+                                              : PrepEntry{(uint32_t)v[c] | (tt << 16), (uint32_t)v[c + 1]};
             if (want && j <= width)
             {
                 store_pair(prep_address + slot * 8u, entry);
@@ -604,8 +612,9 @@
                 const PrepEntry entry = load_pair(pp);
                 const uint64_t ring_words = ring_words_at(ring_address, p);
                 const int rc = kWide ? (int)(entry.x & 0xFFFFu) : (int)(entry.x & 0xFFu);
-                const int rb = (int)entry.y;
-                const int q3 = quantised(rc - a);
+                const int rb = kRelative ? (int)((entry.x >> 8) & 0xFFu) : (int)entry.y;
+                const int ra = kRelative ? (a & 0xFF) : a;
+                const int q3 = quantised(rc - ra);
                 Record updated;
                 {
                     const int n_new = u_n1;
@@ -628,7 +637,7 @@
                 const uint32_t u = lowest_one(win);
                 u1 = u + 1u;
                 const uint32_t beyond = bit_reverse(win >> (u1 & 31u));
-                const int px0 = med3(a + (rb - rc), a, rb);
+                const int px0 = kRelative ? ra + med3((int)entry.y, 0, rb - ra) : med3(a + (rb - rc), a, rb);
                 ok_m = lanes_where(qsu8 != 2912u) & lanes_where(u < limit_v);
                 const int n = (int)(rec.y & 0xFFu);
                 const int cc = (int)(signed char)(rec.y >> 8);
@@ -650,6 +659,8 @@
                     v += v < -near ? range_step : (v > maxval + near ? -range_step : 0);
                     a = med3(v, 0, maxval);
                 }
+                else if (kRelative && maxval == 255)
+                    a = mad24(e, sgn, px);
                 else
                     a = mad24(e, sgn, px) & maxval;
                 k_last = (uint32_t)k;
@@ -729,10 +740,14 @@
                             ok_m |= served_m;
                             const uint32_t may_take = fits ? budget - taken : ~0u;
                             uint32_t left = 63u - (uint32_t)__builtin_clzll(ticker);
+                            const bool first_of_trip = JLS_STEP_TRIP_COUNT != 0 && (left & 1u) != 0;
                             for (LaneMask m = served_m; m != 0;)
                             {
                                 const uint32_t v = value_of_lowest_lane(m, may_take);
-                                left = v < left ? v : left;
+                                uint32_t whole = v;
+                                if (JLS_STEP_TRIP_COUNT != 0)
+                                    whole = first_of_trip ? (v == 0 ? 0u : 1u + ((v - 1u) & ~1u)) : (v & ~1u);
+                                left = whole < left ? whole : left;
                                 m &= ~lanes_where(may_take == v);
                             }
                             ticker = 1ull << left;
@@ -763,6 +778,8 @@
                 ok_m = in_line_m & ~fail_m;
             }
 #endif
+            if (kRelative && !kNear)
+                a &= maxval;
             win_stopped = win_now;
             bool owed_last;
             int ra_stopped;
@@ -1033,7 +1050,8 @@
         if (__any(slow))
         {
             JLS_PATH(9);
-            const int rc = kWide ? (int)(entry_stopped.x & 0xFFFFu) : (int)(entry_stopped.x & 0xFFu), rb = (int)entry_stopped.y;
+            const int rc = kWide ? (int)(entry_stopped.x & 0xFFFFu) : (int)(entry_stopped.x & 0xFFu);
+            const int rb = kRelative ? (int)((entry_stopped.x >> 8) & 0xFFu) : (int)entry_stopped.y;
             const int s = qs8 >> 31;
             const int idx = ((qs8 ^ s) - s) >> 3;
             const Record rec = records[idx];
diff --git a/charls_amd/csrc/device/scan_group_step.inc b/charls_amd/csrc/device/scan_group_step.inc
--- a/charls_amd/csrc/device/scan_group_step.inc
+++ b/charls_amd/csrc/device/scan_group_step.inc
@@ -1,10 +1,49 @@
 
 #define JLS_SDWA(s0, s1) " dst_sel:DWORD dst_unused:UNUSED_PAD src0_sel:" s0 " src1_sel:" s1 "\n"
 
-#define JLS_STEP_PROLOGUE                                                                                                          \
-    "s_mov_b64 s[98:99], exec\n"                                                                                                  \
-    "s_mov_b64 exec, %[inl]\n"                                                                                                    \
-    "ds_read_b64 v[118:119], %[pp] offset:8\n"                                                                                    \
+#ifndef JLS_STEP_MED_FROM_RA
+#define JLS_STEP_MED_FROM_RA 1
+#endif
+
+#ifndef JLS_STEP_TRIP_COUNT
+#define JLS_STEP_TRIP_COUNT 1
+#endif
+#ifndef JLS_STEP_TRIP_POINTERS
+#define JLS_STEP_TRIP_POINTERS 1
+#endif
+#if JLS_STEP_TRIP_POINTERS
+#define JLS_STEP_ADVANCE_A(SZ) ""
+#define JLS_STEP_ADVANCE_B(SZ) "v_add_u32 %[lm], 2 * " SZ ", %[lm]\n v_add_u32 %[pp], 16, %[pp]\n"
+#define JLS_STEP_STORE_OFFSET_A(SZ) " offset:" SZ
+#define JLS_STEP_NEXT_ENTRY_A "16"
+#define JLS_STEP_TRUE_UP_A(SZ) "v_add_u32 %[lm], " SZ ", %[lm]\n v_add_u32 %[pp], 8, %[pp]\n"
+#define JLS_STEP_RARE_ENTER_A(SZ) JLS_STEP_TRUE_UP_A(SZ)
+#define JLS_STEP_RARE_LEAVE_A(SZ) "v_add_u32 %[lm], -" SZ ", %[lm]\n v_add_u32 %[pp], -8, %[pp]\n"
+#else
+#define JLS_STEP_ADVANCE_A(SZ) "v_add_u32 %[lm], " SZ ", %[lm]\n v_add_u32 %[pp], 8, %[pp]\n"
+#define JLS_STEP_ADVANCE_B(SZ) JLS_STEP_ADVANCE_A(SZ)
+#define JLS_STEP_STORE_OFFSET_A(SZ) ""
+#define JLS_STEP_NEXT_ENTRY_A "8"
+#define JLS_STEP_TRUE_UP_A(SZ) ""
+#define JLS_STEP_RARE_ENTER_A(SZ) ""
+#define JLS_STEP_RARE_LEAVE_A(SZ) ""
+#endif
+#define JLS_STEP_TAIL_PER_STEP(DONE, NEXT) "s_sub_u32 %[cnt], %[cnt], 1\n s_cbranch_scc1 " DONE "%=\n" NEXT
+#if JLS_STEP_TRIP_COUNT
+#define JLS_STEP_TAIL_A ""
+#define JLS_STEP_TAIL_B "s_sub_u32 %[cnt], %[cnt], 1\n s_cbranch_scc0 L_stepa%=\n s_branch L_doneb%=\n"
+#define JLS_STEP_BUDGET_A "v_cmp_eq_u32_e64 s[86:87], 0, v89\n v_add_u32 v89, -1, v89\n v_lshrrev_b32 v89, 1, v89\n"
+#define JLS_STEP_BUDGET_B "v_lshrrev_b32 v89, 1, v89\n"
+#define JLS_STEP_SHORT_A "s_cmp_lg_u64 s[86:87], 0\n s_cbranch_scc1 L_doneb%=\n"
+#else
+#define JLS_STEP_TAIL_A JLS_STEP_TAIL_PER_STEP("L_donea", "")
+#define JLS_STEP_TAIL_B JLS_STEP_TAIL_PER_STEP("L_doneb", "s_branch L_stepa%=\n")
+#define JLS_STEP_BUDGET_A ""
+#define JLS_STEP_BUDGET_B ""
+#define JLS_STEP_SHORT_A ""
+#endif
+
+#define JLS_STEP_PROLOGUE_CONSTANTS                                                                                                \
     "v_mov_b32 v100, 0xb60\n"                                                                                                     \
     "v_mov_b32 v101, 0x0c0c0400\n"                                                                                                \
     "v_mov_b32 v103, 0x7f\n"                                                                                                      \
@@ -13,15 +52,38 @@
     "v_mov_b32 v127, 0\n"                                                                                                         \
     "v_lshrrev_b32 v93, 16, %[cfg]\n"                                                                                 \
     "s_waitcnt lgkmcnt(0)\n"
-
-#define JLS_STEP_STORES_LATE(ST) "ds_write2_b32 %[where], %[ua], v111 offset1:1\n", "2", ST " %[lm], %[a]\n", "1"
-#define JLS_STEP_STORES_EARLY(ST) "ds_write2_b32 %[where], %[ua], v111 offset1:1\n" ST " %[lm], %[a]\n", "3", "", "0"
+#define JLS_STEP_PROLOGUE_PER_STEP                                                                                                 \
+    "s_mov_b64 s[98:99], exec\n"                                                                                                  \
+    "s_mov_b64 exec, %[inl]\n"                                                                                                    \
+    "ds_read_b64 v[118:119], %[pp] offset:8\n"                                                                                    \
+    JLS_STEP_PROLOGUE_CONSTANTS
+#if JLS_STEP_TRIP_COUNT
+#define JLS_STEP_PROLOGUE                                                                                                          \
+    "s_mov_b64 s[98:99], exec\n"                                                                                                  \
+    "s_mov_b64 exec, %[inl]\n"                                                                                                    \
+    "s_and_b32 s80, %[cnt], 1\n"                                                                                                  \
+    "s_lshr_b32 %[cnt], %[cnt], 1\n"                                                                                              \
+    "s_cmp_eq_u32 s80, 0\n"                                                                                                       \
+    "s_cbranch_scc1 L_enterb%=\n"                                                                                                 \
+    "ds_read_b64 v[118:119], %[pp] offset:8\n"                                                                                    \
+    JLS_STEP_PROLOGUE_CONSTANTS
+#define JLS_STEP_ENTER_B(SZ)                                                                                                       \
+    "L_enterb%=:\n"                                                                                                               \
+    "ds_read_b64 v[106:107], %[pp] offset:8\n"                                                                                    \
+    JLS_STEP_RARE_LEAVE_A(SZ)                                                         \
+    JLS_STEP_PROLOGUE_CONSTANTS                                                                                                    \
+    "s_branch L_stepb%=\n"
+#else
+#define JLS_STEP_PROLOGUE JLS_STEP_PROLOGUE_PER_STEP
+#define JLS_STEP_ENTER_B(SZ) ""
+#endif
+
+#define JLS_STEP_STORES_LATE(ST, OFF) "ds_write2_b32 %[where], %[ua], v111 offset1:1\n", "2", ST " %[lm], %[a]" OFF "\n", "1"
+#define JLS_STEP_STORES_EARLY(ST, OFF) "ds_write2_b32 %[where], %[ua], v111 offset1:1\n" ST " %[lm], %[a]" OFF "\n", "3", "", "0"
 
 #define JLS_STEP_COMMIT_AND_WINDOW(SZ, TOP_EXTRA) \
      \
     "v_add3_u32 %[p], %[p], %[u1], %[k]\n" \
-    "v_add_u32 %[lm], " SZ ", %[lm]\n" \
-    "v_add_u32 %[pp], 8, %[pp]\n" \
     TOP_EXTRA \
     "v_bfe_u32 v109, %[p], 5, 8\n" \
     "v_lshl_add_u32 v109, v109, 2, %[ring]\n" \
@@ -31,6 +93,10 @@
     "v_add_u32 v115, %[a], " E1 "\n" \
     "v_sub_u32_sdwa v115, v115, " E0 JLS_SDWA("DWORD", RC) \
     "v_med3_i32 v115, v115, %[a], " E1 "\n"
+#define JLS_STEP_PREDICTOR_FROM_RA(RC, E0, E1) \
+    "v_sub_u32_sdwa v115, " E0 ", %[a]" JLS_SDWA("BYTE_1", "BYTE_0") \
+    "v_med3_i32 v115, v115, 0, " E1 "\n" \
+    "v_add_u32_sdwa v115, v115, %[a]" JLS_SDWA("DWORD", "BYTE_0")
 #define JLS_STEP_A13 \
      \
     "v_med3_i32 v110, %[utb], 0, 1\n" \
@@ -58,6 +124,9 @@
     "v_mad_i32_i24 v115, v111, v116, v115\n"                                                                                      \
     "v_and_b32 %[a], %[smax], v115\n"
 #define JLS_STEP_LOSSLESS "", JLS_STEP_ODD_LOSSLESS, JLS_STEP_RECON_LOSSLESS, "v111"
+#define JLS_STEP_RECON_LOSSLESS_BYTE "v_mad_i32_i24 %[a], v111, v116, v115\n"
+#define JLS_STEP_LOSSLESS_BYTE "", JLS_STEP_ODD_LOSSLESS, JLS_STEP_RECON_LOSSLESS_BYTE, "v111"
+#define JLS_STEP_EXIT_BYTE "v_and_b32 %[a], 0xff, %[a]\n"
 #define JLS_STEP_RECON_NEAR                                                                                                        \
     "v_mad_i32_i24 v115, v111, v117, v115\n"                                                                                      \
     "v_cmp_lt_i32 vcc, v115, v96\n"                                                                                               \
@@ -78,17 +147,17 @@
     "v_sub_u32 v97, %[smax], v96\n"                                                                                               \
     "v_sub_u32 v99, 0, v98\n"
 
-#define JLS_STEP_BODY(SFX, NEXT, E0, E1, ENEXT, RC, SZ, BETWEEN, RING_WAIT, AFTER_REQUEST, EARLY_STORES, Q3_WAIT, LATE_STORE, RECORD_WAIT, Q3_ADDR, Q3_OFFSET, TOP_EXTRA, K_EXTRA, A_EXTRA, KSEEN, SIGN_EXTRA, ODD, RECON, UTB_SRC) \
+#define JLS_STEP_BODY(SFX, TAIL, E0, E1, ENEXT, NEXT_OFFSET, RC, ASEL, SZ, BETWEEN, RING_WAIT, AFTER_REQUEST, EARLY_STORES, Q3_WAIT, LATE_STORE, RECORD_WAIT, Q3_ADDR, Q3_OFFSET, TOP_EXTRA, K_EXTRA, A_EXTRA, KSEEN, SIGN_EXTRA, ODD, RECON, UTB_SRC) \
     "L_step" SFX "%=:\n"                                                                                                          \
                                                                 \
-    "v_sub_u32_sdwa v108, " E0 ", %[a]" JLS_SDWA(RC, "DWORD")                                                                    \
+    "v_sub_u32_sdwa v108, " E0 ", %[a]" JLS_SDWA(RC, ASEL)                                                                       \
     Q3_ADDR                                                                                                                       \
     "ds_read_u8 v114, v108" Q3_OFFSET "\n"                                                                            \
     BETWEEN                                                                                                                       \
     EARLY_STORES                                                                                                \
     "s_waitcnt lgkmcnt(" Q3_WAIT ")\n"                                                                           \
     "v_add_u32_sdwa %[qsu], v114, " E0 JLS_SDWA("DWORD", "WORD_1")                                                                \
-    "ds_read_b64 " ENEXT ", %[pp] offset:8\n"                                \
+    "ds_read_b64 " ENEXT ", %[pp] offset:" NEXT_OFFSET "\n"                  \
     "v_sad_u32 %[where], %[qsu], v100, %[recbase]\n"                                                                              \
     "ds_read_b64 v[122:123], %[where]\n"                                                                 \
     LATE_STORE                                                                                                                    \
@@ -130,9 +199,7 @@
     "s_or_b64 s[94:95], s[92:93], s[96:97]\n"                                                    \
     "s_cbranch_scc1 L_rare" SFX "%=\n"                                                                                            \
     "L_back" SFX "%=:\n"                                                                                                          \
-    "s_sub_u32 %[cnt], %[cnt], 1\n"                                                                                               \
-    "s_cbranch_scc1 L_done%=\n"                                                             \
-    NEXT
+    TAIL                                                                                   \
 
 #define JLS_RUN_WHICH_LOSSLESS "v_cmp_eq_u32 s[88:89], v108, v109\n"
 #define JLS_RUN_WHICH_NEAR                                                                                                         \
@@ -150,7 +217,7 @@
     "v_cndmask_b32_e64 v91, v91, v99, s[86:87]\n"                                                                                 \
     "v_add_u32 v112, v112, v91\n"                                                                                                 \
     "v_med3_i32 v112, v112, 0, %[smax]\n"
-#define JLS_STEP_RARE(SFX, LD, ST, SZ, ENEXT, WHICH, RECON)                                                                        \
+#define JLS_STEP_RARE(SFX, LD, ST, SZ, ENEXT, WHICH, RECON, ENTER, LEAVE, BUDGET, SHORT)                                                                      \
     "L_rare" SFX "%=:\n"                                                                                                          \
     "v_cndmask_b32_e64 v108, 0, 1, s[92:93]\n"                                                                                    \
     "v_and_b32 v109, 0xff, v123\n"                                                                                                \
@@ -161,6 +228,7 @@
     "v_add_u32 %[un1], 1, v109\n"                                                                                                 \
     "s_or_b64 %[fail], s[96:97], s[94:95]\n"                                                                                      \
     "s_cbranch_scc0 L_back" SFX "%=\n"                                                              \
+    ENTER                                                                                  \
     "s_cmp_lg_u64 s[96:97], 0\n"                                                                                                  \
     "s_cbranch_scc1 L_exit%=\n"                                              \
                                                                                    \
@@ -313,6 +381,7 @@
     "v_sub_u32_e64 %[ri], v81, 1 clamp\n"                                                         \
                                                         \
     "s_mov_b64 s[82:83], exec\n"                                                                                                  \
+    BUDGET                                                                                                                        \
     "L_budget" SFX "%=:\n"                                                                                                        \
     "s_ff1_i32_b64 s80, s[82:83]\n"                                                                                               \
     "s_nop 3\n"                                                                 \
@@ -327,34 +396,41 @@
     "s_mov_b64 exec, s[90:91]\n"                                                                                                  \
     "s_mov_b64 %[fail], s[94:95]\n"                                                                                               \
     "s_cmp_lg_u64 s[94:95], 0\n"                                                                                                  \
-    "s_cbranch_scc0 L_back" SFX "%=\n"                                                                                            \
-    "s_branch L_exit%=\n"
-
-#define JLS_STEP_EPILOGUE(EXIT_EXTRA)                                                                                              \
-    "L_done%=:\n"                                                                                                                 \
+    "s_cbranch_scc1 L_exit%=\n"                                                                                                   \
+    SHORT                                                                             \
+    LEAVE                                                                                                                         \
+    "s_branch L_back" SFX "%=\n"
+
+#define JLS_STEP_EPILOGUE(EXIT_EXTRA, TRUE_UP_A)                                                                                   \
+    "L_donea%=:\n"                                                                                \
+    TRUE_UP_A                                                                                                                     \
+    "L_doneb%=:\n"                                                                                                                 \
     "s_mov_b64 %[fail], 0\n"                                                                                                      \
     "L_exit%=:\n"                                                                                                                 \
     EXIT_EXTRA                                                                                                                    \
     "s_waitcnt lgkmcnt(0)\n"                                                 \
     "s_mov_b64 exec, s[98:99]\n"
 
-#define JLS_STEP_ORDER_WINDOW_FIRST(RC, SZ, TOP_EXTRA, E0, E1) JLS_STEP_COMMIT_AND_WINDOW(SZ, TOP_EXTRA) JLS_STEP_PREDICTOR(RC, E0, E1) JLS_STEP_A13, "4", ""
-#define JLS_STEP_ORDER_PREDICTOR_LATE(RC, SZ, TOP_EXTRA, E0, E1) JLS_STEP_COMMIT_AND_WINDOW(SZ, TOP_EXTRA) JLS_STEP_A13, "4", JLS_STEP_PREDICTOR(RC, E0, E1)
-#define JLS_STEP_ORDER_UPDATE_FIRST(RC, SZ, TOP_EXTRA, E0, E1)                                                                     \
-    JLS_STEP_A13 "ds_write2_b32 %[where], %[ua], v111 offset1:1\n" JLS_STEP_COMMIT_AND_WINDOW(SZ, TOP_EXTRA) JLS_STEP_PREDICTOR(RC, E0, E1), "3", ""
-#define JLS_STEP_STORES_SAMPLE_LATE(ST) "", "2", ST " %[lm], %[a]\n", "1"
+#define JLS_STEP_ORDER_WINDOW_FIRST(PRED, RC, SZ, TOP_EXTRA, E0, E1) JLS_STEP_COMMIT_AND_WINDOW(SZ, TOP_EXTRA) PRED(RC, E0, E1) JLS_STEP_A13, "4", ""
+#define JLS_STEP_ORDER_PREDICTOR_LATE(PRED, RC, SZ, TOP_EXTRA, E0, E1) JLS_STEP_COMMIT_AND_WINDOW(SZ, TOP_EXTRA) JLS_STEP_A13, "4", PRED(RC, E0, E1)
+#define JLS_STEP_ORDER_UPDATE_FIRST(PRED, RC, SZ, TOP_EXTRA, E0, E1)                                                                    \
+    JLS_STEP_A13 "ds_write2_b32 %[where], %[ua], v111 offset1:1\n" JLS_STEP_COMMIT_AND_WINDOW(SZ, TOP_EXTRA) PRED(RC, E0, E1), "3", ""
+#define JLS_STEP_STORES_SAMPLE_LATE(ST, OFF) "", "2", ST " %[lm], %[a]" OFF "\n", "1"
 #define JLS_STEP_KSEEN "v_or_b32 %[kseen], %[kseen], %[k]\n"
 
 #define JLS_STEP_BODY_X(...) JLS_STEP_BODY(__VA_ARGS__)
-#define JLS_STEP_LOOP_TEXT(RC, SZ, LD, ORDER, STORES, Q3_ADDR, Q3_OFFSET, TOP_EXTRA, K_EXTRA, A_EXTRA, EXIT_EXTRA, MODE, RARE_A, RARE_B)     \
+#define JLS_STEP_LOOP_TEXT(RC, ASEL, PRED, SZ, LD, ORDER, ST, Q3_ADDR, Q3_OFFSET, TOP_EXTRA, K_EXTRA, A_EXTRA, EXIT_EXTRA, MODE, RARE_A, RARE_B)     \
     JLS_STEP_PROLOGUE                                                                                                              \
-    JLS_STEP_BODY_X("a", "", "v118", "v119", "v[106:107]", RC, SZ, ORDER(RC, SZ, TOP_EXTRA, "v118", "v119"), STORES, Q3_ADDR, Q3_OFFSET, TOP_EXTRA, \
-                  K_EXTRA, A_EXTRA, JLS_STEP_KSEEN, MODE)                                                                          \
-    JLS_STEP_BODY_X("b", "s_branch L_stepa%=\n", "v106", "v107", "v[118:119]", RC, SZ, ORDER(RC, SZ, TOP_EXTRA, "v106", "v107"), STORES, Q3_ADDR, \
+    JLS_STEP_BODY_X("a", JLS_STEP_TAIL_A, "v118", "v119", "v[106:107]", JLS_STEP_NEXT_ENTRY_A, RC, ASEL, SZ,                      \
+                  ORDER(PRED, RC, SZ, JLS_STEP_ADVANCE_A(SZ) TOP_EXTRA, "v118", "v119"), JLS_STEP_STORES_LATE(ST, JLS_STEP_STORE_OFFSET_A(SZ)), \
+                  Q3_ADDR, Q3_OFFSET, TOP_EXTRA, K_EXTRA, A_EXTRA, JLS_STEP_KSEEN, MODE)                                           \
+    JLS_STEP_BODY_X("b", JLS_STEP_TAIL_B, "v106", "v107", "v[118:119]", "8", RC, ASEL, SZ,                                        \
+                  ORDER(PRED, RC, SZ, JLS_STEP_ADVANCE_B(SZ) TOP_EXTRA, "v106", "v107"), JLS_STEP_STORES_LATE(ST, ""), Q3_ADDR,    \
                   Q3_OFFSET, TOP_EXTRA, K_EXTRA, A_EXTRA, JLS_STEP_KSEEN, MODE)                                                    \
+    JLS_STEP_ENTER_B(SZ)                                                                                                           \
     RARE_A                                                                                                                         \
     RARE_B                                                                                                                         \
-    JLS_STEP_EPILOGUE(EXIT_EXTRA)
+    JLS_STEP_EPILOGUE(EXIT_EXTRA, JLS_STEP_TRUE_UP_A(SZ))
 
 #define JLS_STEP_LOOP_CLOBBERS                                                                                                     \
     "memory", "vcc", "scc", "s80", "s81", "s82", "s83", "s84", "s85", "s86", "s87", "s88", "s89", "s90", "s91", "s92", "s93", "s94", "s95", "s96",   \
@@ -362,8 +438,11 @@
         "v108", "v109", "v110", "v111", "v112", "v113", "v114", "v115", "v116", "v117", "v118", "v119", "v120", "v121", "v122", "v123", "v124",  \
         "v125", "v126", "v127"
 
-#define JLS_STEP_RARE_NARROW(SFX, ENEXT, WHICH, RECON) JLS_STEP_RARE(SFX, "ds_read_u8", "ds_write_b8", "1", ENEXT, WHICH, RECON)
-#define JLS_STEP_RARE_WIDE(SFX, ENEXT, WHICH, RECON) JLS_STEP_RARE(SFX, "ds_read_u16", "ds_write_b16", "2", ENEXT, WHICH, RECON)
+#define JLS_STEP_RARE_A(LD, ST, SZ, WHICH, RECON)                                                                                 \
+    JLS_STEP_RARE("a", LD, ST, SZ, "v[106:107]", WHICH, RECON, JLS_STEP_RARE_ENTER_A(SZ), JLS_STEP_RARE_LEAVE_A(SZ), JLS_STEP_BUDGET_A, JLS_STEP_SHORT_A)
+#define JLS_STEP_RARE_B(LD, ST, SZ, WHICH, RECON) JLS_STEP_RARE("b", LD, ST, SZ, "v[118:119]", WHICH, RECON, "", "", JLS_STEP_BUDGET_B, "")
+#define JLS_STEP_RARE_NARROW(SFX, WHICH, RECON) JLS_STEP_RARE_##SFX("ds_read_u8", "ds_write_b8", "1", WHICH, RECON)
+#define JLS_STEP_RARE_WIDE(SFX, WHICH, RECON) JLS_STEP_RARE_##SFX("ds_read_u16", "ds_write_b16", "2", WHICH, RECON)
 #define JLS_STEP_OPERANDS_OUT                                                                                                      \
     [a] "+v"(a), [p] "+v"(p), [lm] "+v"(lm), [pp] "+v"(pp), [where] "+v"(where), [ua] "+v"(u_a), [un1] "+v"(u_n1), [utb] "+v"(u_tb), \
         [cc] "+v"(u_cc), [u1] "+v"(u1), [k] "+v"(k_last), [kseen] "+v"(k_seen), [qsu] "+v"(qsu8), [win] "+v"(win_now),             \
@@ -373,13 +452,39 @@
     [ring] "v"(ring_address), [recbase] "v"(records_address), [limitv] "v"(limit_v), [cfg] "v"(cfg_v), [inl] "s"(in_line_m),       \
         [smax] "s"(maxval_s), [rctx] "v"(run_ctx_address), [gl] "n"(G)
 
-#define JLS_STEP_LOOP_ASM_NARROW()                                                                                                 \
-    asm volatile(JLS_STEP_LOOP_TEXT("BYTE_0", "1", "ds_read_u8", JLS_STEP_ORDER_WINDOW_FIRST,                                      \
-                                    JLS_STEP_STORES_LATE("ds_write_b8"), "", " offset:255", "", "", "", "", JLS_STEP_LOSSLESS,      \
-                                    JLS_STEP_RARE_NARROW("a", "v[106:107]", JLS_RUN_WHICH_LOSSLESS, JLS_RUN_RECON_LOSSLESS), JLS_STEP_RARE_NARROW("b", "v[118:119]", JLS_RUN_WHICH_LOSSLESS, JLS_RUN_RECON_LOSSLESS))                          \
+#if JLS_STEP_MED_FROM_RA
+#define JLS_STEP_NARROW_ASEL "BYTE_0"
+#define JLS_STEP_NARROW_PRED JLS_STEP_PREDICTOR_FROM_RA
+#else
+#define JLS_STEP_NARROW_ASEL "DWORD"
+#define JLS_STEP_NARROW_PRED JLS_STEP_PREDICTOR
+#endif
+#define JLS_STEP_LOOP_ASM_NARROW_MASKED()                                                                                          \
+    asm volatile(JLS_STEP_LOOP_TEXT("BYTE_0", JLS_STEP_NARROW_ASEL, JLS_STEP_NARROW_PRED, "1", "ds_read_u8", JLS_STEP_ORDER_WINDOW_FIRST, \
+                                    "ds_write_b8", "", " offset:255", "", "", "", "", JLS_STEP_LOSSLESS,      \
+                                    JLS_STEP_RARE_NARROW(A, JLS_RUN_WHICH_LOSSLESS, JLS_RUN_RECON_LOSSLESS), JLS_STEP_RARE_NARROW(B, JLS_RUN_WHICH_LOSSLESS, JLS_RUN_RECON_LOSSLESS))                          \
                  : JLS_STEP_OPERANDS_OUT                                                                                           \
                  : JLS_STEP_OPERANDS_IN                                                                                            \
                  : JLS_STEP_LOOP_CLOBBERS)
+#if JLS_STEP_MED_FROM_RA
+#define JLS_STEP_LOOP_ASM_NARROW()                                                                                                 \
+    do                                                                                                                             \
+    {                                                                                                                              \
+        if (maxval_s == 255)                                                                                                       \
+            asm volatile(JLS_STEP_LOOP_TEXT("BYTE_0", "BYTE_0", JLS_STEP_PREDICTOR_FROM_RA, "1", "ds_read_u8", JLS_STEP_ORDER_WINDOW_FIRST, \
+                                            "ds_write_b8", "", " offset:255", "", "", "", JLS_STEP_EXIT_BYTE, \
+                                            JLS_STEP_LOSSLESS_BYTE,                                                                \
+                                            JLS_STEP_RARE_NARROW(A, JLS_RUN_WHICH_LOSSLESS, JLS_RUN_RECON_LOSSLESS), \
+                                            JLS_STEP_RARE_NARROW(B, JLS_RUN_WHICH_LOSSLESS, JLS_RUN_RECON_LOSSLESS)) \
+                         : JLS_STEP_OPERANDS_OUT                                                                                   \
+                         : JLS_STEP_OPERANDS_IN                                                                                    \
+                         : JLS_STEP_LOOP_CLOBBERS);                                                                                \
+        else                                                                                                                       \
+            JLS_STEP_LOOP_ASM_NARROW_MASKED();                                                                                     \
+    } while (0)
+#else
+#define JLS_STEP_LOOP_ASM_NARROW() JLS_STEP_LOOP_ASM_NARROW_MASKED()
+#endif
 
 #define JLS_STEP_CHECKED_TOP "v_or_b32 %[mmseen], %[mmseen], v127\n"
 #define JLS_STEP_CHECKED_K "v_add_u32 v112, v125, %[k]\n v_cmp_le_u32 vcc, 32, v112\n s_or_b64 s[96:97], s[96:97], vcc\n"
@@ -388,27 +493,27 @@
 #define JLS_STEP_WIDE_Q3 "v_med3_i32 v108, v108, v102, %[vcap]\n v_add_u32 v108, %[vcap], v108\n"
 #define JLS_STEP_LOOP_ASM_WIDE()                                                                                                   \
     asm volatile("v_sub_u32 v102, 0, %[vcap]\n"                                                                                   \
-                 JLS_STEP_LOOP_TEXT("WORD_0", "2", "ds_read_u16", JLS_STEP_ORDER_WINDOW_FIRST, JLS_STEP_STORES_LATE("ds_write_b16"), \
+                 JLS_STEP_LOOP_TEXT("WORD_0", "DWORD", JLS_STEP_PREDICTOR, "2", "ds_read_u16", JLS_STEP_ORDER_WINDOW_FIRST, "ds_write_b16", \
                                     JLS_STEP_WIDE_Q3, "", JLS_STEP_CHECKED_TOP, JLS_STEP_CHECKED_K, JLS_STEP_CHECKED_A,             \
                                     JLS_STEP_CHECKED_EXIT, JLS_STEP_LOSSLESS,                                                      \
-                                    JLS_STEP_RARE_WIDE("a", "v[106:107]", JLS_RUN_WHICH_LOSSLESS, JLS_RUN_RECON_LOSSLESS), JLS_STEP_RARE_WIDE("b", "v[118:119]", JLS_RUN_WHICH_LOSSLESS, JLS_RUN_RECON_LOSSLESS))                            \
+                                    JLS_STEP_RARE_WIDE(A, JLS_RUN_WHICH_LOSSLESS, JLS_RUN_RECON_LOSSLESS), JLS_STEP_RARE_WIDE(B, JLS_RUN_WHICH_LOSSLESS, JLS_RUN_RECON_LOSSLESS))                            \
                  : JLS_STEP_OPERANDS_OUT JLS_STEP_OPERANDS_CHECKED                                                                 \
                  : JLS_STEP_OPERANDS_IN, [vcap] "v"(cap_v)                                                                         \
                  : JLS_STEP_LOOP_CLOBBERS)
 
 #define JLS_STEP_LOOP_ASM_NARROW_NEAR()                                                                                            \
     asm volatile(JLS_STEP_NEAR_CONSTANTS                                                                                           \
-                 JLS_STEP_LOOP_TEXT("BYTE_0", "1", "ds_read_u8", JLS_STEP_ORDER_WINDOW_FIRST, JLS_STEP_STORES_LATE("ds_write_b8"), \
+                 JLS_STEP_LOOP_TEXT("BYTE_0", JLS_STEP_NARROW_ASEL, JLS_STEP_NARROW_PRED, "1", "ds_read_u8", JLS_STEP_ORDER_WINDOW_FIRST, "ds_write_b8", \
                                     "", " offset:255", JLS_STEP_CHECKED_TOP, JLS_STEP_CHECKED_K, JLS_STEP_CHECKED_A,                \
-                                    JLS_STEP_CHECKED_EXIT, JLS_STEP_NEAR, JLS_STEP_RARE_NARROW("a", "v[106:107]", JLS_RUN_WHICH_NEAR, JLS_RUN_RECON_NEAR), JLS_STEP_RARE_NARROW("b", "v[118:119]", JLS_RUN_WHICH_NEAR, JLS_RUN_RECON_NEAR)) \
+                                    JLS_STEP_CHECKED_EXIT, JLS_STEP_NEAR, JLS_STEP_RARE_NARROW(A, JLS_RUN_WHICH_NEAR, JLS_RUN_RECON_NEAR), JLS_STEP_RARE_NARROW(B, JLS_RUN_WHICH_NEAR, JLS_RUN_RECON_NEAR)) \
                  : JLS_STEP_OPERANDS_OUT JLS_STEP_OPERANDS_CHECKED                                                                 \
                  : JLS_STEP_OPERANDS_IN, [nr] "s"(near_range_s)                                                                    \
                  : JLS_STEP_LOOP_CLOBBERS)
 #define JLS_STEP_LOOP_ASM_WIDE_NEAR()                                                                                              \
     asm volatile("v_sub_u32 v102, 0, %[vcap]\n" JLS_STEP_NEAR_CONSTANTS                                                           \
-                 JLS_STEP_LOOP_TEXT("WORD_0", "2", "ds_read_u16", JLS_STEP_ORDER_WINDOW_FIRST, JLS_STEP_STORES_LATE("ds_write_b16"), \
+                 JLS_STEP_LOOP_TEXT("WORD_0", "DWORD", JLS_STEP_PREDICTOR, "2", "ds_read_u16", JLS_STEP_ORDER_WINDOW_FIRST, "ds_write_b16", \
                                     JLS_STEP_WIDE_Q3, "", JLS_STEP_CHECKED_TOP, JLS_STEP_CHECKED_K, JLS_STEP_CHECKED_A,             \
-                                    JLS_STEP_CHECKED_EXIT, JLS_STEP_NEAR, JLS_STEP_RARE_WIDE("a", "v[106:107]", JLS_RUN_WHICH_NEAR, JLS_RUN_RECON_NEAR), JLS_STEP_RARE_WIDE("b", "v[118:119]", JLS_RUN_WHICH_NEAR, JLS_RUN_RECON_NEAR)) \
+                                    JLS_STEP_CHECKED_EXIT, JLS_STEP_NEAR, JLS_STEP_RARE_WIDE(A, JLS_RUN_WHICH_NEAR, JLS_RUN_RECON_NEAR), JLS_STEP_RARE_WIDE(B, JLS_RUN_WHICH_NEAR, JLS_RUN_RECON_NEAR)) \
                  : JLS_STEP_OPERANDS_OUT JLS_STEP_OPERANDS_CHECKED                                                                 \
                  : JLS_STEP_OPERANDS_IN, [vcap] "v"(cap_v), [nr] "s"(near_range_s)                                                 \
                  : JLS_STEP_LOOP_CLOBBERS)
```

Result: faster. 18260 (median of 6 runs) (+3.9%).
